# jasperlinthorst/reveal

Hardware: AMD Instinct MI355X
Metric: Mbp/s indexed+MUM-anchored (reveal rem) (higher is better)
Workload: dtype int32

## Files before the change

include/reveal_amd.h:

```cpp
#ifndef REVEAL_AMD_H
#define REVEAL_AMD_H
#include <stdint.h>

#ifdef __cplusplus
extern "C" {
#endif

typedef struct rv_index rv_index;

const char *rv_last_error(void);
int  rv_abi_version(void);
int  rv_sa_bits(void);
int  rv_device_count(void);

rv_index *rv_new(int device);
void rv_free(rv_index *h);

int rv_add_sample(rv_index *h);
int rv_add_sequence(rv_index *h, const char *seq, int64_t len, int64_t *begin, int64_t *end);
int rv_reset(rv_index *h);
int rv_reserve_text(rv_index *h, int64_t bytes);
int64_t rv_n(const rv_index *h);
int rv_nsamples(const rv_index *h);
int rv_nnodes(const rv_index *h);
int rv_add_sequences(rv_index *h, const char *text, int64_t total, const int64_t *lens, int64_t count);
int rv_node_list(const rv_index *h, int64_t *begin_end);

int rv_construct(rv_index *h, int rc, const char *safile, const char *lcpfile, int cache);
int rv_upload(rv_index *h);
int rv_upload_again(rv_index *h);

enum { RV_T = 0, RV_SA = 1, RV_SAI = 2, RV_LCP = 3, RV_SO = 4, RV_NSEP = 5, RV_NODES = 6 };
int64_t rv_get_array(rv_index *h, int which, void *out, int64_t cap);

int64_t rv_getmums(rv_index *h, int minl);
int rv_fetch_mums(rv_index *h, uint32_t *l, int64_t *a, int64_t *b, int64_t cap);
int64_t rv_getmultimums(rv_index *h, int minlength, int minn, int mems, int64_t *members);
int rv_fetch_multi(rv_index *h, uint32_t *l, int32_t *n, int64_t *off, uint16_t *so, int64_t *pos);

typedef struct {
    int64_t n;
    int32_t depth;
    int32_t nsamples;
    int32_t nnodes;
    int32_t parent;
    int32_t kind;
    int32_t reserved;
    int64_t nmums;
    int64_t nmembers;
} rv_sub;

int rv_align_begin(rv_index *h, int minl, int minn);
int rv_frontier_size(rv_index *h);
int rv_frontier_scan(rv_index *h);
int rv_sub_skip_scan(rv_index *h, int s);
int rv_sub_info(rv_index *h, int s, rv_sub *out);
int rv_sub_nodes(rv_index *h, int s, int64_t *begin_end );
int rv_sub_mums(rv_index *h, int s, uint32_t *l, int32_t *n, int64_t *off, uint16_t *so, int64_t *pos);
int64_t rv_sub_array(rv_index *h, int s, int which, void *out, int64_t cap);
int rv_sub_split(rv_index *h, int s, uint32_t l, int nsp, const int64_t *sp,
                 const int64_t *lead, int nlead, const int64_t *trail, int ntrail,
                 const int64_t *match, int nmatch, const int64_t *rest, int nrest);
int rv_frontier_commit(rv_index *h, int32_t *children);
int rv_align_end(rv_index *h);

typedef struct {
    int64_t steps;
    int64_t splits;
    int64_t anchored_bp;
    int32_t levels;
    int32_t maxdepth;
    int64_t scanned_ranks;
    double  t_scan, t_host, t_split, t_bubble;
} rv_align_stats;
int rv_align_builtin(rv_index *h, int minl, int minn, rv_align_stats *st);

int rv_align_builtin_until(rv_index *h, int minl, int minn, int stop_subs, rv_align_stats *st);
int rv_align_builtin_resume(rv_index *h, rv_align_stats *st);
int rv_align_builtin_continue(rv_index *h, int stop_subs, rv_align_stats *st);
int rv_frontier_counts(rv_index *h, int64_t *out);
int rv_frontier_export(rv_index *h, int64_t *meta, int64_t *node_first, int64_t *nodes);
int64_t rv_frontier_pack(rv_index *h, const int32_t *subs, int k, void *sa, void *lcp, void *bwt, int on_device);
int rv_frontier_import(rv_index *h, int minl, int minn, uint32_t maxlcp, int level, int nsubs, const int64_t *meta,
                       const int64_t *node_first, const int64_t *nodes, int64_t m,
                       const void *sa, const void *lcp, const void *bwt, int on_device);
int64_t rv_frontier_seeds_export(rv_index *h, const int32_t *subs, int k, int64_t *out, int64_t cap);
int rv_frontier_seeds_import(rv_index *h, int nsubs, const int64_t *words, int64_t nwords);
uint32_t rv_maxlcp(const rv_index *h);
int rv_cascade_info(const rv_index *h, int64_t *out);
const char *rv_cascade_why(const rv_index *h);
int64_t rv_anchor_count(rv_index *h, int64_t *members);
int rv_fetch_anchors(rv_index *h, uint32_t *l, int64_t *off, int64_t *pos);
int rv_set_result_buffers(rv_index *h, uint32_t *l, int64_t l_cap, int64_t *off, int64_t off_cap, int64_t *pos, int64_t pos_cap);
typedef struct {
    int64_t  key, n;
    int32_t  depth, nsamples, nnodes, picked;
    int64_t  nmums;
    uint32_t l; int32_t mn;
    int64_t  sp_min;
    uint64_t h_sa, h_lcp, h_mums;
} rv_trace;
int rv_set_trace(rv_index *h, int on);
int rv_set_preselect(rv_index *h, int64_t maxmums);
int rv_set_option(rv_index *h, const char *name, int64_t value);
int rv_get_option(rv_index *h, const char *name, int64_t *value);
int rv_set_launch_trace(int on);
int rv_option_count(void);
const char *rv_option_name(int k);
int64_t rv_trace_count(rv_index *h);
int rv_fetch_trace(rv_index *h, rv_trace *out, int64_t cap);

typedef struct rv_subindex rv_subindex;
rv_index *rv_clone(rv_index *h);
rv_subindex *rv_sx_main(rv_index *h);
rv_subindex *rv_sx_copy(rv_subindex *x);
void rv_sx_free(rv_subindex *x);
int rv_sx_info(const rv_subindex *x, rv_sub *out);
int rv_sx_nodes(const rv_subindex *x, int64_t *begin_end);
int64_t rv_sx_array(rv_subindex *x, int which, void *out, int64_t cap);
int64_t rv_sx_scan(rv_subindex *x, int minl, int minn, int64_t *members);
int rv_sx_fetch(rv_subindex *x, uint32_t *l, int32_t *n, int64_t *off, uint16_t *so, int64_t *pos);
int rv_sx_split(rv_subindex *x, const int64_t *lead, int nlead, const int64_t *trail, int ntrail,
                const int64_t *match, int nmatch, const int64_t *rest, int nrest, rv_subindex **out);
int rv_sx_extract(rv_subindex *x, int64_t *intervals, int niv);

int64_t rv_chain(int64_t m, int k, const uint32_t *len, const int32_t *nmem, const int64_t *crd, const int64_t *left,
                 const int64_t *right, int64_t wscore, int64_t wpen, int model, int64_t *out_idx, int64_t *out_score);

typedef struct { int64_t wscore, wpen, maxmums, seedsize; int gcmodel; int trim; double pcutoff; } rv_picker_args;
typedef struct {
    int picked; uint32_t pick_l; int32_t pick_n; int pick_members; uint16_t *pick_so; int64_t *pick_pos; int64_t member_cap;
    int64_t nleft, nright, nseed_members, seed_cap, seed_member_cap;
    uint32_t *seed_l; int32_t *seed_n; int64_t *seed_off; uint16_t *seed_so; int64_t *seed_pos; int64_t *seed_score; uint8_t *seed_right;
} rv_picker_out;
int rv_set_picker(rv_index *h, int kind, const rv_picker_args *args);
int rv_picker_info(const rv_index *h, int64_t *out);
int rv_pick_chain(const rv_picker_args *args, int nsub, int64_t m, const uint32_t *l, const int32_t *n, const int64_t *off, const uint16_t *so,
                  const int64_t *pos, int nsamples, const int64_t *seq_begin, const int64_t *iv_begin, const int64_t *iv_end, int minlength,
                  rv_picker_out *out);

typedef struct rv_graph rv_graph;
rv_graph *rv_graph_import(int64_t nnodes, const int64_t *node_b, const int64_t *node_e, const int8_t *node_aligned, const int8_t *node_sent,
                          const int64_t *off_ptr, const int32_t *off_sid, const int64_t *off_val,
                          int64_t nedges, const int32_t *edge_u, const int32_t *edge_v, const int64_t *edge_ptr, const int32_t *edge_paths,
                          const int64_t *pred_ptr, const int32_t *pred_edge, int npaths, const uint8_t *star, const int64_t *id2end,
                          int nstart, const int32_t *start_nodes, int literal_segments);
int rv_graph_pick(rv_graph *g, const rv_picker_args *args, int nsub, int64_t m, const uint32_t *l, const int32_t *n, const int64_t *off, const uint16_t *so, const int64_t *pos,
                  const int64_t *left, const int64_t *right, int minlength, rv_picker_out *out);
int rv_graph_align(rv_graph *g, const int64_t *nodes, int64_t nn, const int64_t *left, const int64_t *right, uint32_t l, const int64_t *pos, int npos,
                   int64_t *counts, int64_t *out6);
int rv_graph_align_fetch(rv_graph *g, int64_t *out);
int rv_set_graph_picker(rv_index *h, rv_graph *g, const rv_picker_args *args);
rv_graph *rv_graph_new(void);
int rv_graph_add_linear(rv_graph *g, int64_t b, int64_t e, int star);
int64_t rv_graph_read_gfa(rv_graph *g, rv_index *h, int64_t *text_n, const char *data, int64_t len, const char **names);
typedef struct GfaParsed rv_gfa_parsed;
rv_gfa_parsed *rv_gfa_parse(const char *data, int64_t len);
int64_t rv_graph_adopt(rv_graph *g, rv_index *h, int64_t *text_n, rv_gfa_parsed *parsed, const char **names);
void rv_gfa_parsed_free(rv_gfa_parsed *parsed);
int rv_graph_seal(rv_graph *g);
int rv_graph_paths(const rv_graph *g, int64_t *id2end);
int rv_graph_node_kinds(const rv_graph *g, int8_t *out);
int rv_graph_literal(const rv_graph *g);
int rv_graph_finish(rv_graph *g);
rv_graph *rv_graph_replay_begin(int nseq, const int64_t *begin, const int64_t *end);
int rv_set_replay_graph(rv_index *h, rv_graph *g);
rv_graph *rv_graph_replay(int nseq, const int64_t *begin, const int64_t *end, int64_t na, const uint32_t *an_l, const int64_t *an_off, const int64_t *an_pos);
const char *rv_graph_error(const rv_graph *g);
int rv_graph_sizes(const rv_graph *g, int64_t *out);
int rv_graph_export(const rv_graph *g, int64_t *node_b, int64_t *node_e, int8_t *node_aligned, int64_t *off_ptr, int32_t *off_sid, int64_t *off_val,
                    int64_t *succ_ptr, int32_t *succ_to, int32_t *succ_edge, int64_t *pred_ptr, int32_t *pred_from, int32_t *pred_edge, int64_t *edge_ptr, int32_t *edge_paths);
int rv_graph_prune(rv_graph *g, const char *T);
int64_t rv_graph_gfa(rv_graph *g, const char *T, int npaths, const char *const *names, const char *cmdline, const char **out);
void rv_graph_free(rv_graph *g);

enum { RV_K_SCAN_PAIR = 0, RV_K_SCAN_MULTI = 1, RV_K_SA_SORT = 2, RV_K_LCP = 3, RV_K_SPLIT = 4, RV_K_LABEL = 5,
       RV_K_BUBBLE = 6,
       RV_K_RADIX_SCATTER = 7, RV_K_RADIX_HIST = 8, RV_K_TEXT_ROUND = 9,
       RV_K_CASCADE = 10,
       RV_K_DIAG_TABLE = 11,
       RV_K_INIT_KEYS = 12,
       RV_K_PUBLISH = 13,
       RV_K_COUNT = 14 };
int rv_prof_enable(rv_index *h, int on);
int rv_prof_reset(rv_index *h);
int rv_prof_get(rv_index *h, int k, int64_t *launches, double *ms, double *bytes);
typedef struct rv_batch rv_batch;
rv_batch *rv_batch_new(void);
int rv_batch_add(rv_batch *b, rv_index *h);
int rv_batch_run(rv_batch *b, int minl, int minn, int construct, rv_align_stats *stats, int *status);
int rv_batch_info(const rv_batch *b, int64_t *out);
void rv_batch_free(rv_batch *b);
typedef struct rv_many rv_many;
rv_many *rv_many_new(int device);
void rv_many_free(rv_many *m);
int rv_many_option(rv_many *m, const char *name, int64_t value);
int64_t rv_many_add(rv_many *m, const char *const *seqs, const int64_t *lens, int k);
int rv_many_clear(rv_many *m);
int rv_many_run(rv_many *m, int minl, int minn, rv_align_stats *total);
int64_t rv_many_anchor_count(rv_many *m, int64_t *first, int64_t *members);
int rv_many_fetch(rv_many *m, uint32_t *l, int64_t *off, int64_t *pos);
int64_t rv_many_text(rv_many *m, int64_t job, char *out, int64_t cap);
int rv_many_info(const rv_many *m, int64_t *out);
int64_t rv_many_arrays(rv_many *m, int64_t job, int which, void *out, int64_t cap);
void *rv_dev_alloc(int device, int64_t bytes);
int rv_dev_free(int device, void *p);
int rv_ipc_export(int device, const void *p, uint8_t handle[64]);
void *rv_ipc_open(int device, const uint8_t handle[64]);
int rv_ipc_close(int device, void *p);
int rv_dev_copy(int device, void *dst, const void *src, int64_t bytes);
int rv_measure_bandwidth(int device, int64_t bytes, int iters, double *read_gbs, double *copy_gbs);
int rv_sa_stats(rv_index *h, int *sigma, int *bits, int *k0, int *rounds, int64_t *sorted_elems, int *radix_passes);
int rv_sa_diag_table(rv_index *h);
int rv_sa_tail(rv_index *h, int64_t *out);

int rv_test_exclusive_sum_u32(const uint32_t *in, uint32_t *out, int64_t n);
int rv_test_inclusive_max_u32(const uint32_t *in, uint32_t *out, int64_t n);
int rv_test_radix_sort(uint64_t *keys, uint32_t *vals, int64_t n, int bit_lo, int bit_hi);
int rv_test_radix_time(int64_t n, int bits, int dist, int flags, int iters, double *ms, int64_t *bad);

#ifdef __cplusplus
}
#endif
#endif
```

reveal_amd/_lib.py:

```python
import ctypes
import importlib.util
import os
import sys
import numpy as np

_HERE = os.path.dirname(os.path.abspath(__file__))

RV_T, RV_SA, RV_SAI, RV_LCP, RV_SO, RV_NSEP, RV_NODES = range(7)
K_SCAN_PAIR, K_SCAN_MULTI, K_SA_SORT, K_LCP, K_SPLIT, K_LABEL, K_BUBBLE, K_RADIX_SCATTER, K_RADIX_HIST, K_TEXT_ROUND, K_CASCADE, K_DIAG_TABLE, K_INIT_KEYS, K_PUBLISH = range(14)

c_i64p = ctypes.POINTER(ctypes.c_int64)
V = ctypes.c_void_p


class RvSub(ctypes.Structure):
    _fields_ = [("n", ctypes.c_int64), ("depth", ctypes.c_int32), ("nsamples", ctypes.c_int32),
                ("nnodes", ctypes.c_int32), ("parent", ctypes.c_int32), ("kind", ctypes.c_int32),
                ("reserved", ctypes.c_int32), ("nmums", ctypes.c_int64), ("nmembers", ctypes.c_int64)]


class RvAlignStats(ctypes.Structure):
    _fields_ = [("steps", ctypes.c_int64), ("splits", ctypes.c_int64), ("anchored_bp", ctypes.c_int64),
                ("levels", ctypes.c_int32), ("maxdepth", ctypes.c_int32), ("scanned_ranks", ctypes.c_int64),
                ("t_scan", ctypes.c_double), ("t_host", ctypes.c_double), ("t_split", ctypes.c_double),
                ("t_bubble", ctypes.c_double)]


TRACE_DTYPE = np.dtype([("key", np.int64), ("n", np.int64), ("depth", np.int32), ("nsamples", np.int32),
                        ("nnodes", np.int32), ("picked", np.int32), ("nmums", np.int64), ("l", np.uint32),
                        ("mn", np.int32), ("sp_min", np.int64), ("h_sa", np.uint64), ("h_lcp", np.uint64),
                        ("h_mums", np.uint64)], align=True)

_I, _L, _D = ctypes.c_int, ctypes.c_int64, ctypes.c_double
SYMBOLS = {
    "rv_last_error": (ctypes.c_char_p, []),
    "rv_abi_version": (_I, []),
    "rv_sa_bits": (_I, []),
    "rv_device_count": (_I, []),
    "rv_new": (V, [_I]),
    "rv_free": (None, [V]),
    "rv_add_sample": (_I, [V]),
    "rv_add_sequence": (_I, [V, ctypes.c_char_p, _L, c_i64p, c_i64p]),
    "rv_reset": (_I, [V]),
    "rv_reserve_text": (_I, [V, _L]),
    "rv_n": (_L, [V]),
    "rv_nsamples": (_I, [V]),
    "rv_nnodes": (_I, [V]),
    "rv_node_list": (_I, [V, V]),
    "rv_construct": (_I, [V, _I, ctypes.c_char_p, ctypes.c_char_p, _I]),
    "rv_upload": (_I, [V]),
    "rv_upload_again": (_I, [V]),
    "rv_get_array": (_L, [V, _I, V, _L]),
    "rv_getmums": (_L, [V, _I]),
    "rv_fetch_mums": (_I, [V, V, V, V, _L]),
    "rv_getmultimums": (_L, [V, _I, _I, _I, c_i64p]),
    "rv_fetch_multi": (_I, [V, V, V, V, V, V]),
    "rv_align_begin": (_I, [V, _I, _I]),
    "rv_frontier_size": (_I, [V]),
    "rv_frontier_scan": (_I, [V]),
    "rv_sub_skip_scan": (_I, [V, _I]),
    "rv_sub_info": (_I, [V, _I, ctypes.POINTER(RvSub)]),
    "rv_sub_nodes": (_I, [V, _I, V]),
    "rv_sub_mums": (_I, [V, _I, V, V, V, V, V]),
    "rv_sub_array": (_L, [V, _I, _I, V, _L]),
    "rv_sub_split": (_I, [V, _I, ctypes.c_uint32, _I, V, V, _I, V, _I, V, _I, V, _I]),
    "rv_frontier_commit": (_I, [V, V]),
    "rv_align_end": (_I, [V]),
    "rv_align_builtin": (_I, [V, _I, _I, ctypes.POINTER(RvAlignStats)]),
    "rv_align_builtin_until": (_I, [V, _I, _I, _I, ctypes.POINTER(RvAlignStats)]),
    "rv_align_builtin_resume": (_I, [V, ctypes.POINTER(RvAlignStats)]),
    "rv_align_builtin_continue": (_I, [V, _I, ctypes.POINTER(RvAlignStats)]),
    "rv_frontier_counts": (_I, [V, V]),
    "rv_frontier_export": (_I, [V, V, V, V]),
    "rv_frontier_pack": (_L, [V, V, _I, V, V, V, _I]),
    "rv_frontier_import": (_I, [V, _I, _I, ctypes.c_uint32, _I, _I, V, V, V, _L, V, V, V, _I]),
    "rv_frontier_seeds_export": (_L, [V, V, _I, V, _L]),
    "rv_frontier_seeds_import": (_I, [V, _I, V, _L]),
    "rv_maxlcp": (ctypes.c_uint32, [V]),
    "rv_cascade_info": (ctypes.c_int, [V, V]),
    "rv_cascade_why": (ctypes.c_char_p, [V]),
    "rv_anchor_count": (_L, [V, c_i64p]),
    "rv_fetch_anchors": (_I, [V, V, V, V]),
    "rv_set_result_buffers": (_I, [V, V, _L, V, _L, V, _L]),
    "rv_set_trace": (_I, [V, _I]),
    "rv_set_preselect": (_I, [V, _L]),
    "rv_set_option": (_I, [V, ctypes.c_char_p, _L]),
    "rv_set_launch_trace": (_I, [_I]),
    "rv_batch_new": (V, []),
    "rv_batch_add": (_I, [V, V]),
    "rv_batch_run": (_I, [V, _I, _I, _I, V, V]),
    "rv_batch_info": (_I, [V, V]),
    "rv_batch_free": (None, [V]),
    "rv_dev_alloc": (V, [_I, _L]),
    "rv_dev_free": (_I, [_I, V]),
    "rv_ipc_export": (_I, [_I, V, V]),
    "rv_ipc_open": (V, [_I, V]),
    "rv_ipc_close": (_I, [_I, V]),
    "rv_dev_copy": (_I, [_I, V, V, _L]),
    "rv_get_option": (_I, [V, ctypes.c_char_p, c_i64p]),
    "rv_option_count": (_I, []),
    "rv_option_name": (ctypes.c_char_p, [_I]),
    "rv_trace_count": (_L, [V]),
    "rv_fetch_trace": (_I, [V, V, _L]),
    "rv_clone": (V, [V]),
    "rv_sx_main": (V, [V]),
    "rv_sx_copy": (V, [V]),
    "rv_sx_free": (None, [V]),
    "rv_sx_info": (_I, [V, ctypes.POINTER(RvSub)]),
    "rv_sx_nodes": (_I, [V, V]),
    "rv_sx_array": (_L, [V, _I, V, _L]),
    "rv_sx_scan": (_L, [V, _I, _I, c_i64p]),
    "rv_sx_fetch": (_I, [V, V, V, V, V, V]),
    "rv_sx_split": (_I, [V, V, _I, V, _I, V, _I, V, _I, V]),
    "rv_sx_extract": (_I, [V, V, _I]),
    "rv_chain": (_L, [_L, _I, V, V, V, V, V, _L, _L, _I, V, V]),
    "rv_prof_enable": (_I, [V, _I]),
    "rv_prof_reset": (_I, [V]),
    "rv_prof_get": (_I, [V, _I, c_i64p, ctypes.POINTER(_D), ctypes.POINTER(_D)]),
    "rv_measure_bandwidth": (_I, [_I, _L, _I, ctypes.POINTER(_D), ctypes.POINTER(_D)]),
    "rv_sa_stats": (_I, [V] + [ctypes.POINTER(_I)] * 4 + [c_i64p, ctypes.POINTER(_I)]),
    "rv_sa_diag_table": (_I, [V]),
    "rv_sa_tail": (_I, [V, c_i64p]),
    "rv_set_picker": (_I, [V, _I, V]),
    "rv_picker_info": (_I, [V, c_i64p]),
    "rv_pick_chain": (_I, [V, _I, _L, V, V, V, V, V, _I, V, V, V, _I, V]),
    "rv_graph_import": (V, [_L, V, V, V, V, V, V, V, _L, V, V, V, V, V, V, _I, V, V, _I, V, _I]),
    "rv_graph_pick": (_I, [V, V, _I, _L, V, V, V, V, V, V, V, _I, V]),
    "rv_graph_align": (_I, [V, V, _L, V, V, ctypes.c_uint32, V, _I, V, V]),
    "rv_graph_align_fetch": (_I, [V, V]),
    "rv_graph_finish": (_I, [V]),
    "rv_set_graph_picker": (_I, [V, V, V]),
    "rv_graph_new": (V, []),
    "rv_graph_replay_begin": (V, [_I, V, V]),
    "rv_set_replay_graph": (_I, [V, V]),
    "rv_graph_add_linear": (_I, [V, _L, _L, _I]),
    "rv_graph_read_gfa": (_L, [V, V, V, V, _L, V]),
    "rv_graph_paths": (_I, [V, V]),
    "rv_graph_seal": (_I, [V]),
    "rv_gfa_parse": (V, [V, _L]),
    "rv_graph_adopt": (_L, [V, V, V, V, V]),
    "rv_gfa_parsed_free": (None, [V]),
    "rv_add_sequences": (_I, [V, V, _L, V, _L]),
    "rv_graph_node_kinds": (_I, [V, V]),
    "rv_graph_literal": (_I, [V]),
    "rv_graph_replay": (V, [_I, V, V, _L, V, V, V]),
    "rv_graph_error": (ctypes.c_char_p, [V]),
    "rv_graph_sizes": (_I, [V, c_i64p]),
    "rv_graph_export": (_I, [V] * 15),
    "rv_graph_prune": (_I, [V, V]),
    "rv_graph_gfa": (_L, [V, V, _I, V, V, V]),
    "rv_graph_free": (None, [V]),
    "rv_many_new": (V, [_I]),
    "rv_many_free": (None, [V]),
    "rv_many_option": (_I, [V, ctypes.c_char_p, _L]),
    "rv_many_add": (_L, [V, V, V, _I]),
    "rv_many_clear": (_I, [V]),
    "rv_many_run": (_I, [V, _I, _I, ctypes.POINTER(RvAlignStats)]),
    "rv_many_anchor_count": (_L, [V, V, c_i64p]),
    "rv_many_fetch": (_I, [V, V, V, V]),
    "rv_many_text": (_L, [V, _L, V, _L]),
    "rv_many_info": (_I, [V, V]),
    "rv_many_arrays": (_L, [V, _L, _I, V, _L]),
    "rv_test_exclusive_sum_u32": (_I, [V, V, _L]),
    "rv_test_inclusive_max_u32": (_I, [V, V, _L]),
    "rv_test_radix_sort": (_I, [V, V, _L, _I, _I]),
    "rv_test_radix_time": (_I, [_L, _I, _I, _I, _I, ctypes.POINTER(_D), c_i64p]),
}


def _share_torch_runtime():
    if os.environ.get("RV_SYSTEM_HIP") or "torch" in sys.modules:
        return
    try:
        spec = importlib.util.find_spec("torch")
    except (ImportError, ValueError):
        spec = None
    if spec is None or not spec.origin:
        return
    path = os.path.join(os.path.dirname(spec.origin), "lib", "libamdhip64.so")
    if os.path.exists(path):
        ctypes.CDLL(path, mode=ctypes.RTLD_GLOBAL)


class Lib:
    def __init__(self, sa64=False):
        self.sa64 = sa64
        _share_torch_runtime()
        name = "libreveal_amd64.so" if sa64 else "libreveal_amd.so"
        self.path = os.path.join(os.environ.get("RV_LIB_DIR") or _HERE, name)
        if not os.path.exists(self.path):
            raise ImportError("%s is missing: build it with `python -c 'import __graft_entry__ as g; g.build()'` "
                              "(hipcc --offload-arch=gfx950); reveal_amd has no CPU fallback" % self.path)
        self.dll = ctypes.CDLL(self.path)
        for sym, (res, args) in SYMBOLS.items():
            fn = getattr(self.dll, sym)
            fn.restype, fn.argtypes = res, args
        self.sa_t = np.int64 if sa64 else np.int32
        self.lcp_t = np.uint32 if sa64 else np.int32
        assert self.dll.rv_sa_bits() == (64 if sa64 else 32)
        v = os.environ.get("RV_LAUNCH_TRACE")
        if v is not None and v.strip() not in ("", "0"):
            self.dll.rv_set_launch_trace(1)

    def err(self):
        return (self.dll.rv_last_error() or b"").decode(errors="replace")


_libs = {}
_device = 0


def set_device(i):
    global _device
    _device = int(i)


def device():
    return _device


def measure_bandwidth(nbytes=1 << 30, iters=10):
    lib = get(False)
    r, c = _D(0), _D(0)
    if lib.dll.rv_measure_bandwidth(device(), int(nbytes), int(iters), ctypes.byref(r), ctypes.byref(c)) != 0:
        raise RuntimeError(lib.err())
    return r.value, c.value


def set_launch_trace(on=True):
    return [bool(get(w).dll.rv_set_launch_trace(1 if on else 0)) for w in (False, True)]


def get(sa64=False):
    if sa64 not in _libs:
        _libs[sa64] = Lib(sa64)
    return _libs[sa64]
```

reveal_amd/csrc/rv_api.hip:

```cpp
#include "rv_index.h"
#include "rv_cascade.h"
#include <limits>
#include <stdarg.h>
#include <stdio.h>
#include <string.h>
#include <limits.h>
#include <algorithm>
#include <thread>

static thread_local char g_err[1024] = "";

void rv_set_error(const char *fmt, ...) {
    va_list ap;
    va_start(ap, fmt);
    vsnprintf(g_err, sizeof g_err, fmt, ap);
    va_end(ap);
}

static std::vector<rv_index *> &live_handles() { static std::vector<rv_index *> v; return v; }
std::mutex &rv_trim_mutex() { static std::mutex *m = new std::mutex(); return *m; }
bool rv_oom_trim() {
    size_t got = 0;
    bool log = false;
    int caller_dev = 0;
// ... 844 lines not shown
int64_t rv_getmums(rv_index *h, int minl) {
    if (!h->constructed || h->main_arrays_freed) { rv_set_error("Index not yet constructed."); return -2; }
    (void)hipSetDevice(h->device);
    std::vector<RvPairRec> recs;
    if (rv_run_pair_scan(h, h->dSA.as<sa_t>(), h->dLCP.as<lcp_t>(), h->dBWT.as<uint8_t>(), h->n, minl, recs, nullptr, nullptr, nullptr, 0, nullptr, false) != 0) return -1;
    h->m_l.resize(recs.size()); h->m_a.resize(recs.size()); h->m_b.resize(recs.size());
    for (size_t k = 0; k < recs.size(); k++) {
        int64_t b = recs[k].b;
        if (h->rc == 1) b = h->nsep[0] + (h->nT - b - (int64_t)recs[k].l);
        h->m_l[k] = recs[k].l; h->m_a[k] = recs[k].a; h->m_b[k] = b;
    }
    return (int64_t)recs.size();
}

int rv_fetch_mums(rv_index *h, uint32_t *l, int64_t *a, int64_t *b, int64_t cap) {
    if (cap < (int64_t)h->m_l.size()) { rv_set_error("buffer too small"); return -1; }
    for (size_t k = 0; k < h->m_l.size(); k++) { l[k] = h->m_l[k]; a[k] = h->m_a[k]; b[k] = h->m_b[k]; }
    return 0;
}

int rv_prof_enable(rv_index *h, int on) {
    h->prof.on = on != 0;
    h->prof.mask = (on & 1) ? 0xFFFFFFFFu : ((u32)on >> 1);
    return 0;
}
int rv_prof_reset(rv_index *h) { (void)hipStreamSynchronize(h->ws.stream); h->prof.reset(); return 0; }
int rv_prof_get(rv_index *h, int k, int64_t *launches, double *ms, double *bytes) {
    if (k < 0 || k >= RV_K_COUNT) { rv_set_error("bad kernel id"); return -1; }
    (void)hipStreamSynchronize(h->ws.stream);
    h->prof.resolve();
    if (launches) *launches = h->prof.launches[k];
    if (ms) *ms = h->prof.ms[k];
    if (bytes) *bytes = h->prof.bytes[k];
    return 0;
}
int rv_sa_stats(rv_index *h, int *sigma, int *bits, int *k0, int *rounds, int64_t *sorted_elems, int *radix_passes) {
    if (sigma) *sigma = h->sa_stats.sigma;
    if (bits) *bits = h->sa_stats.bits;
    if (k0) *k0 = h->sa_stats.k0;
    if (rounds) *rounds = h->sa_stats.rounds;
    if (sorted_elems) *sorted_elems = h->sa_stats.sorted_elems;
    if (radix_passes) *radix_passes = h->sa_stats.radix_passes;
    return 0;
}
int rv_sa_diag_table(rv_index *h) { return h->sa_stats.diag_table; }
int rv_sa_tail(rv_index *h, int64_t *out) { if (!h || !out) return -1; out[0] = h->sa_stats.far_pairs; out[1] = h->sa_stats.lcp_list; return 0; }

}
namespace {
typedef int bw_v4 __attribute__((ext_vector_type(4)));
__global__ __launch_bounds__(256) void k_bw_read(const bw_v4 *__restrict__ a, int64_t n16, unsigned *sink) {
    bw_v4 acc = {0, 0, 0, 0};
    for (int64_t i = (int64_t)blockIdx.x * 256 + threadIdx.x; i < n16; i += (int64_t)gridDim.x * 256) acc ^= __builtin_nontemporal_load(a + i);
    if ((acc.x ^ acc.y ^ acc.z ^ acc.w) == 0x12345678) sink[0] = 1;
}
__global__ __launch_bounds__(256) void k_bw_copy(const bw_v4 *__restrict__ a, bw_v4 *__restrict__ b, int64_t n16) {
    for (int64_t i = (int64_t)blockIdx.x * 256 + threadIdx.x; i < n16; i += (int64_t)gridDim.x * 256) __builtin_nontemporal_store(__builtin_nontemporal_load(a + i), b + i);
}
}
extern "C" {
struct rv_batch {
    std::vector<rv_index *> hs;
    RvBatchGroup *g = nullptr;
    std::vector<std::string> errs;
};
rv_batch *rv_batch_new(void) {
    try { return new rv_batch(); } catch (...) { rv_set_error("rv_batch_new: out of host memory"); return nullptr; }
}
int rv_batch_add(rv_batch *b, rv_index *h) {
    if (!b || !h) { rv_set_error("rv_batch_add: null argument"); return -1; }
    if (!b->hs.empty() && b->hs[0]->device != h->device) { rv_set_error("rv_batch_add: the handles of a batch live on one device"); return -1; }
    try { b->hs.push_back(h); } catch (...) { rv_set_error("rv_batch_add: out of host memory"); return -1; }
    return 0;
}
void rv_batch_free(rv_batch *b) {
    if (!b) return;
    rv_batch_group_free(b->g);
    delete b;
}
int rv_batch_info(const rv_batch *b, int64_t *out) {
    out[0] = out[1] = 0;
    if (b && b->g) rv_batch_group_info(b->g, out);
    return 0;
}
int rv_batch_run(rv_batch *b, int minl, int minn, int construct, rv_align_stats *stats, int *status) {
    if (!b || b->hs.empty()) { rv_set_error("rv_batch_run: empty batch"); return -1; }
    const int n = (int)b->hs.size();
    try {
        b->errs.assign((size_t)n, std::string());
        if (!b->g) b->g = rv_batch_group_new(b->hs[0]->device);
        int members = 0;
        for (rv_index *h : b->hs) {
            const bool in = h->nsamples > 2 && !h->ws.opt.no_cascade;
            h->batch = in ? b->g : nullptr; h->batch_settled = false;
            members += in ? 1 : 0;
        }
        rv_batch_group_begin(b->g, members);
        std::vector<int> rc((size_t)n, 0);
        auto work = [&](int i) {
            rv_index *h = b->hs[(size_t)i];
            int r = 0;
            if (hipSetDevice(h->device) != hipSuccess) { rv_set_error("hipSetDevice failed"); r = -1; }
            if (r == 0 && construct) r = rv_construct(h, 0, "", "", 0);
            if (r == 0) r = rv_align_builtin(h, minl, minn, stats ? &stats[i] : nullptr);
            if (h->batch && !h->batch_settled) { h->batch_settled = true; rv_batch_group_leave(h->batch); }
            if (r != 0) b->errs[(size_t)i] = rv_last_error();
            rc[(size_t)i] = r;
        };
        std::vector<std::thread> th;
        int started = n;
        for (int i = 1; i < n; i++) {
            try { th.emplace_back(work, i); }
            catch (...) { started = i; break; }
        }
        if (started < n) for (int i = started; i < n; i++) { rv_index *h = b->hs[(size_t)i]; if (h->batch) { h->batch_settled = true; rv_batch_group_leave(h->batch); h->batch = nullptr; } }
        work(0);
        for (auto &t : th) t.join();
        for (int i = started; i < n; i++) work(i);
        int bad = -1;
        for (int i = 0; i < n; i++) { b->hs[(size_t)i]->batch = nullptr; if (status) status[i] = rc[(size_t)i]; if (rc[(size_t)i] != 0 && bad < 0) bad = i; }
        if (bad >= 0) { rv_set_error("rv_batch_run: job %d: %s", bad, b->errs[(size_t)bad].c_str()); return -1; }
        return 0;
    } catch (const std::exception &e) {
        for (rv_index *h : b->hs) h->batch = nullptr;
        rv_set_error("rv_batch_run: %s", e.what());
        return -1;
    }
}

void *rv_dev_alloc(int device, int64_t bytes) {
    void *p = nullptr;
    if (bytes < 0 || hipSetDevice(device) != hipSuccess) { rv_set_error("rv_dev_alloc: bad device or size"); return nullptr; }
    const hipError_t e = hipMalloc(&p, (size_t)std::max<int64_t>(bytes, 256));
    if (e != hipSuccess) { (void)hipGetLastError(); rv_set_error("rv_dev_alloc(%lld bytes): %s", (long long)bytes, hipGetErrorString(e)); return nullptr; }
    return p;
}
int rv_dev_free(int device, void *p) {
    if (!p) return 0;
    RV_HIP(hipSetDevice(device));
    RV_HIP(hipFree(p));
    return 0;
}
int rv_ipc_export(int device, const void *p, uint8_t handle[64]) {
    static_assert(sizeof(hipIpcMemHandle_t) == 64, "hipIpcMemHandle_t is 64 bytes");
    RV_HIP(hipSetDevice(device));
    hipIpcMemHandle_t hd;
    RV_HIP(hipIpcGetMemHandle(&hd, const_cast<void *>(p)));
    memcpy(handle, &hd, 64);
    return 0;
}
void *rv_ipc_open(int device, const uint8_t handle[64]) {
    if (hipSetDevice(device) != hipSuccess) { rv_set_error("rv_ipc_open: bad device"); return nullptr; }
    hipIpcMemHandle_t hd;
    memcpy(&hd, handle, 64);
    void *p = nullptr;
    const hipError_t e = hipIpcOpenMemHandle(&p, hd, hipIpcMemLazyEnablePeerAccess);
    if (e != hipSuccess) { (void)hipGetLastError(); rv_set_error("rv_ipc_open: %s", hipGetErrorString(e)); return nullptr; }
    return p;
}
int rv_ipc_close(int device, void *p) {
    if (!p) return 0;
    RV_HIP(hipSetDevice(device));
    RV_HIP(hipIpcCloseMemHandle(p));
    return 0;
}
int rv_dev_copy(int device, void *dst, const void *src, int64_t bytes) {
    if (bytes <= 0) return 0;
    RV_HIP(hipSetDevice(device));
    RV_HIP(hipMemcpy(dst, src, (size_t)bytes, hipMemcpyDefault));
    RV_HIP(hipStreamSynchronize(nullptr));
    return 0;
}

int rv_measure_bandwidth(int device, int64_t bytes, int iters, double *read_gbs, double *copy_gbs) {
    if (bytes < (1 << 20) || iters < 1) { rv_set_error("rv_measure_bandwidth: bytes >= 1 MiB and iters >= 1 needed"); return -1; }
    RV_HIP(hipSetDevice(device));
    const int64_t n16 = bytes / 16;
    void *a = nullptr, *b = nullptr; unsigned *sink = nullptr;
    hipStream_t q = nullptr; hipEvent_t e0 = nullptr, e1 = nullptr;
    RV_HIP(hipMalloc(&a, (size_t)n16 * 16)); RV_HIP(hipMalloc(&b, (size_t)n16 * 16)); RV_HIP(hipMalloc((void **)&sink, 64));
    RV_HIP(hipStreamCreateWithFlags(&q, hipStreamNonBlocking));
    RV_HIP(hipEventCreate(&e0)); RV_HIP(hipEventCreate(&e1));
    RV_HIP(hipMemsetAsync(a, 1, (size_t)n16 * 16, q)); RV_HIP(hipMemsetAsync(b, 2, (size_t)n16 * 16, q));
    const unsigned grid = 256 * 16;
    double out[2] = {0, 0};
    for (int pass = 0; pass < 2; pass++) {
        for (int r = -1; r < iters; r++) {
            if (r == 0) RV_HIP(hipEventRecord(e0, q));
            if (pass == 0) hipLaunchKernelGGL(k_bw_read, dim3(grid), dim3(256), 0, q, (const bw_v4 *)a, n16, sink);
            else hipLaunchKernelGGL(k_bw_copy, dim3(grid), dim3(256), 0, q, (const bw_v4 *)a, (bw_v4 *)b, n16);
        }
        RV_HIP(hipEventRecord(e1, q));
        RV_HIP(hipEventSynchronize(e1));
        float ms = 0.f;
        RV_HIP(hipEventElapsedTime(&ms, e0, e1));
        out[pass] = (double)n16 * 16 * (pass ? 2 : 1) * iters / ((double)ms * 1e6);
    }
    if (read_gbs) *read_gbs = out[0];
    if (copy_gbs) *copy_gbs = out[1];
    (void)hipEventDestroy(e0); (void)hipEventDestroy(e1); (void)hipStreamDestroy(q);
    (void)hipFree(a); (void)hipFree(b); (void)hipFree(sink);
    return 0;
}

static int test_ws(Workspace &ws) {
    if (rv_device_count() <= 0) { rv_set_error("no HIP device"); return -1; }
    RV_HIP(hipSetDevice(0));
    RV_HIP(hipStreamCreateWithFlags(&ws.stream, hipStreamNonBlocking));
    return 0;
}
static void test_ws_done(Workspace &ws) { ws.release(); (void)hipStreamDestroy(ws.stream); }

static int test_scan(const uint32_t *in, uint32_t *out, int64_t n, bool maxscan) {
    Workspace ws;
    RV_TRY(test_ws(ws));
    DBuf a, b;
    int r = 0;
    if (a.reserve((size_t)n * 4 + 64) || b.reserve((size_t)n * 4 + 64)) r = -1;
    if (!r && hipMemcpy(a.p, in, (size_t)n * 4, hipMemcpyHostToDevice) != hipSuccess) r = -1;
    if (!r) r = maxscan ? rv_inclusive_max_u32(ws, a.as<u32>(), b.as<u32>(), n) : rv_exclusive_sum_u32(ws, a.as<u32>(), b.as<u32>(), n);
    if (!r && hipStreamSynchronize(ws.stream) != hipSuccess) { rv_set_error("sync failed: %s", hipGetErrorString(hipGetLastError())); r = -1; }
    if (!r && hipMemcpy(out, b.p, (size_t)n * 4, hipMemcpyDeviceToHost) != hipSuccess) r = -1;
    a.release(); b.release();
    test_ws_done(ws);
    return r;
}
int rv_test_exclusive_sum_u32(const uint32_t *in, uint32_t *out, int64_t n) { return test_scan(in, out, n, false); }
int rv_test_inclusive_max_u32(const uint32_t *in, uint32_t *out, int64_t n) { return test_scan(in, out, n, true); }

int rv_test_radix_sort(uint64_t *keys, uint32_t *vals, int64_t n, int bit_lo, int bit_hi) {
    Workspace ws;
    RV_TRY(test_ws(ws));
    DBuf k0, k1, v0, v1;
    int r = 0, in1 = 0;
    if (k0.reserve((size_t)n * 8 + 64) || k1.reserve((size_t)n * 8 + 64) || v0.reserve((size_t)n * 4 + 64) || v1.reserve((size_t)n * 4 + 64)) r = -1;
    if (!r && hipMemcpy(k0.p, keys, (size_t)n * 8, hipMemcpyHostToDevice) != hipSuccess) r = -1;
    if (!r && hipMemcpy(v0.p, vals, (size_t)n * 4, hipMemcpyHostToDevice) != hipSuccess) r = -1;
    if (!r) r = rv_radix_sort_pairs<u32>(ws, k0.as<u64>(), v0.as<u32>(), k1.as<u64>(), v1.as<u32>(), n, bit_lo, bit_hi, &in1);
    if (!r && hipStreamSynchronize(ws.stream) != hipSuccess) { rv_set_error("sync failed: %s", hipGetErrorString(hipGetLastError())); r = -1; }
    if (!r && hipMemcpy(keys, in1 ? k1.p : k0.p, (size_t)n * 8, hipMemcpyDeviceToHost) != hipSuccess) r = -1;
    if (!r && hipMemcpy(vals, in1 ? v1.p : v0.p, (size_t)n * 4, hipMemcpyDeviceToHost) != hipSuccess) r = -1;
    k0.release(); k1.release(); v0.release(); v1.release();
    test_ws_done(ws);
    return r;
}

}
namespace {
__device__ inline u64 rt_mix(u64 x) { x ^= x >> 33; x *= 0xff51afd7ed558ccdull; x ^= x >> 33; x *= 0xc4ceb9fe1a85ec53ull; x ^= x >> 33; return x; }
__global__ __launch_bounds__(256) void k_rt_fill(u64 *keys, u32 *vals, int64_t n, int bits, int dist) {
    const int64_t i = (int64_t)blockIdx.x * 256 + threadIdx.x;
    if (i >= n) return;
    u64 r = rt_mix((u64)i * 0x9E3779B97F4A7C15ull + 12345);
    u64 k = 0;
    if (dist == 0) k = r;
    else if (dist == 1) { u64 r2 = rt_mix(r); for (int j = 0; j < 17; j++) { k = k * 5 + 1 + (r2 & 3); r2 >>= 2; } }
    const u64 mask = bits >= 64 ? ~0ull : (1ull << bits) - 1;
    keys[i] = (k & mask) | (r & ~mask & 0x00ffffffffffffffull);
    vals[i] = (u32)i;
}
__global__ __launch_bounds__(256) void k_rt_check(const u64 *keys, const u32 *vals, int64_t n, int bits, unsigned long long *bad) {
    const int64_t i = (int64_t)blockIdx.x * 256 + threadIdx.x;
    if (i + 1 >= n) return;
    const u64 mask = bits >= 64 ? ~0ull : (1ull << bits) - 1;
    const u64 a = keys[i] & mask, b = keys[i + 1] & mask;
    if (a > b || (a == b && vals[i] > vals[i + 1])) atomicAdd(bad, 1ull);
}
}
extern "C" {
int rv_test_radix_time(int64_t n, int bits, int dist, int flags, int iters, double *ms, int64_t *bad) {
    Workspace ws;
    RV_TRY(test_ws(ws));
    ws.opt.rs_bits = (flags & 1) ? 10 : 8; ws.opt.rs_xcd = (flags & 2) ? 1 : 0; ws.opt.rs_cnt16 = (flags & 4) ? 1 : 0; ws.opt.rs_no_digit_bytes = (flags & 8) ? 1 : 0;
    DBuf k0, k1, v0, v1, db;
    int r = 0, in1 = 0;
    hipEvent_t e0 = nullptr, e1 = nullptr;
    if (k0.reserve((size_t)n * 8 + 64) || k1.reserve((size_t)n * 8 + 64) || v0.reserve((size_t)n * 4 + 64) || v1.reserve((size_t)n * 4 + 64) || db.reserve(64)) r = -1;
    if (!r && (hipEventCreate(&e0) != hipSuccess || hipEventCreate(&e1) != hipSuccess)) r = -1;
    for (int it = 0; !r && it < iters; it++) {
        hipLaunchKernelGGL(k_rt_fill, dim3((unsigned)ceil_div(n, 256)), dim3(256), 0, ws.stream, k0.as<u64>(), v0.as<u32>(), n, bits, dist);
        (void)hipEventRecord(e0, ws.stream);
        r = rv_radix_sort_pairs<u32>(ws, k0.as<u64>(), v0.as<u32>(), k1.as<u64>(), v1.as<u32>(), n, 0, bits, &in1);
        (void)hipEventRecord(e1, ws.stream);
        if (!r && hipEventSynchronize(e1) != hipSuccess) { rv_set_error("sync failed: %s", hipGetErrorString(hipGetLastError())); r = -1; }
        float t = 0;
        if (!r) { (void)hipEventElapsedTime(&t, e0, e1); ms[it] = t; }
    }
    if (!r) {
        (void)hipMemsetAsync(db.p, 0, 8, ws.stream);
        hipLaunchKernelGGL(k_rt_check, dim3((unsigned)ceil_div(n, 256)), dim3(256), 0, ws.stream, (const u64 *)(in1 ? k1.p : k0.p), (const u32 *)(in1 ? v1.p : v0.p), n, bits,
                           db.as<unsigned long long>());
        unsigned long long b = 0;
        if (hipMemcpyAsync(&b, db.p, 8, hipMemcpyDeviceToHost, ws.stream) != hipSuccess || hipStreamSynchronize(ws.stream) != hipSuccess) r = -1;
        *bad = (int64_t)b;
    }
    if (e0) (void)hipEventDestroy(e0);
    if (e1) (void)hipEventDestroy(e1);
    k0.release(); k1.release(); v0.release(); v1.release(); db.release();
    test_ws_done(ws);
    return r;
}

}
```

reveal_amd/csrc/rv_common.h:

```cpp
#pragma once
#include <mutex>
#include <thread>
#include <vector>
#include <utility>
#include <hip/hip_runtime.h>
#include <stdint.h>
#include <string.h>
#include <stddef.h>
#include <vector>
#include <string>

#ifdef RV_SA64
typedef int64_t  sa_t;
typedef uint32_t lcp_t;
#else
typedef int32_t  sa_t;
typedef int32_t  lcp_t;
#endif

typedef unsigned long long u64;
typedef unsigned int       u32;

void rv_set_error(const char *fmt, ...);

#define RV_HIP(x)                                                                              \
    do {                                                                                       \
        hipError_t e_ = (x);                                                                   \
        if (e_ != hipSuccess) {                                                                \
            rv_set_error("%s:%d %s: %s", __FILE__, __LINE__, #x, hipGetErrorString(e_));       \
            return -1;                                                                         \
        }                                                                                      \
    } while (0)
#define RV_TRY(x)                                                                              \
    do {                                                                                       \
        int r_ = (x);                                                                          \
        if (r_ != 0) return r_;                                                                \
    } while (0)
#define RV_OPTION_LIST(X) \
    X(bubble_par_min, "RV_BUBBLE_PAR_MIN", -1) \
    X(presel_log, "RV_PRESEL_LOG", 0) \
    X(presel_host, "RV_PRESEL_HOST", 0) \
    X(leaf_acap, "RV_LEAF_ACAP", 256) \
    X(bubble_lds_always, "RV_BUBBLE_LDS_ALWAYS", 0) \
    X(no_early_bubble, "RV_NO_EARLY_BUBBLE", 0) \
    X(early_bubble_many, "RV_EARLY_BUBBLE_MANY", 0) \
    X(no_early_split, "RV_NO_EARLY_SPLIT", 0) \
    X(keep_dead, "RV_KEEP_DEAD", 0) \
    X(bubble_no_lds, "RV_BUBBLE_NO_LDS", 0) \
    X(bubble_no_join, "RV_BUBBLE_NO_JOIN", 0) \
    X(bubble_no_merge, "RV_BUBBLE_NO_MERGE", 0) \
    X(tables_memcpy, "RV_TABLES_MEMCPY", 0) \
    X(bubble_parent_scratch, "RV_BUBBLE_PARENT_SCRATCH", 0) \
    X(level_log, "RV_LEVEL_LOG", 0) \
    X(pb_two_pass, "RV_PB_TWO_PASS", 0) \
    X(no_leaf, "RV_NO_LEAF", 0) \
    X(leaf_prof, "RV_LEAF_PROF", 0) \
    X(no_cascade, "RV_NO_CASCADE", 0) \
    X(cascade_second, "RV_CASCADE_SECOND", 0) \
    X(cascade_danger, "RV_CASCADE_DANGER", 1) \
    X(cascade_second_off, "RV_CASCADE_SECOND_OFF", 0) \
    X(sync_block, "RV_SYNC_BLOCK", 0) \
    X(pb_refresh_tmin, "RV_PB_REFRESH_TMIN", 0) \
    X(cascade_log, "RV_CASCADE_LOG", 0) \
    X(cascade_danger_min, "RV_CASCADE_DANGER_MIN", 0) \
    X(cascade_batch, "RV_CASCADE_BATCH", 8) \
    X(lcp_by_rank, "RV_LCP_BY_RANK", 0) \
    X(no_tiny_sa, "RV_NO_TINY_SA", 0) \
    X(no_short_alphabet, "RV_NO_SHORT_ALPHABET", 0) \
    X(no_fused_lcp, "RV_NO_FUSED_LCP", 0) \
    X(no_diag, "RV_NO_DIAG", 0) \
    X(no_packed_text, "RV_NO_PACKED_TEXT", 0) \
    X(no_heads_fusion, "RV_NO_HEADS_FUSION", 0) \
    X(no_twin_collapse, "RV_NO_TWIN_COLLAPSE", 0) \
    X(no_far_twins, "RV_NO_FAR_TWINS", 0) \
    X(no_lcp_list, "RV_NO_LCP_LIST", 0) \
    X(no_text_jump, "RV_NO_TEXT_JUMP", 0) \
    X(far_table, "RV_FAR_TABLE", 0) \
    X(no_slow_class, "RV_NO_SLOW_CLASS", 0) \
    X(no_dwalk_blocks, "RV_NO_DWALK_BLOCKS", 0) \
    X(no_pub_twins, "RV_NO_PUB_TWINS", 0) \
    X(sa_no_text, "RV_SA_NO_TEXT", 0) \
    X(text_mode, "RV_TEXT_MODE", -1) \
    X(carry_ch, "RV_CARRY_CH", -1) \
    X(rs_bits, "RV_RS_BITS", 8) \
    X(rs_xcd, "RV_RS_XCD", 1) \
    X(rs_cnt16, "RV_RS_CNT16", 1) \
    X(rs_no_digit_bytes, "RV_RS_NO_DIGIT_BYTES", 0) \
    X(diag_table, "RV_DIAG_TABLE", -1) \
    X(no_cascade_chain, "RV_NO_CASCADE_CHAIN", 0) \
    X(casm_rank_count, "RV_CASM_RANK_COUNT", 0) \
    X(casm_big_min, "RV_CASM_BIG_MIN", -1) \
    X(casm_no_big, "RV_CASM_NO_BIG", 0) \
    X(casm_big_root, "RV_CASM_BIG_ROOT", 1 << 22) \
    X(casm_big_total, "RV_CASM_BIG_TOTAL", 1 << 26) \
    X(lock_any, "RV_LOCK_ANY", 0) \
    X(presel_dev_min, "RV_PRESEL_DEV_MIN", 65536) \
    X(scan_v1, "RV_SCAN_V1", 0) \
    X(pick_threads, "RV_PICK_THREADS", 0) \
    X(cascade_prio, "RV_CASCADE_PRIO", 0)
struct RvOptions {
#define RV_X_(f, name, def) int64_t f = def;
    RV_OPTION_LIST(RV_X_)
#undef RV_X_
    int64_t *find(const char *name) {
#define RV_X_(f, nm, def) if (strcmp(name, nm) == 0) return &f;
        RV_OPTION_LIST(RV_X_)
#undef RV_X_
        return nullptr;
    }
};
extern int g_rv_launch_trace;
static inline bool rv_launch_trace_on() { return g_rv_launch_trace != 0; }
#define RV_LAUNCH_CHECK()                                                                      \
    do {                                                                                       \
        RV_HIP(hipGetLastError());                                                             \
        if (rv_launch_trace_on()) {                                                            \
            fprintf(stderr, "launch %s:%d\n", __FILE__, __LINE__);                             \
            fflush(stderr);                                                                    \
            RV_HIP(hipDeviceSynchronize());                                                    \
        }                                                                                      \
    } while (0)

static inline int64_t ceil_div(int64_t a, int64_t b) { return (a + b - 1) / b; }

#define RV_BWT_SIDE 0x80u
#define RV_BWT_CHAR 0x7fu

#ifdef __HIPCC__
__device__ inline u32 rv_wave_min_u32(u32 v) {
    const int inf = -1;
    int x = (int)v, y;
#define RV_DPP_MIN(ctrl, rmask)                                                        \
    y = __builtin_amdgcn_update_dpp(inf, x, ctrl, rmask, 0xf, false);                  \
    x = (int)(((u32)y < (u32)x) ? (u32)y : (u32)x);
    RV_DPP_MIN(0xB1, 0xf)
    RV_DPP_MIN(0x4E, 0xf)
    RV_DPP_MIN(0x141, 0xf)
    RV_DPP_MIN(0x140, 0xf)
    RV_DPP_MIN(0x142, 0xa)
    RV_DPP_MIN(0x143, 0xc)
#undef RV_DPP_MIN
    return (u32)__builtin_amdgcn_readlane(x, 63);
}
#endif

#ifdef __HIPCC__
template <int CTRL, int ROWMASK> __device__ inline u32 rv_dpp_u32(u32 x) { return (u32)__builtin_amdgcn_update_dpp(0, (int)x, CTRL, ROWMASK, 0xf, false); }
#define RV_WAVE_SCAN_STEPS(STEP)                                                     \
    STEP(0x111, 0xf, (lane & 15) >= 1)                                               \
    STEP(0x112, 0xf, (lane & 15) >= 2)                                               \
    STEP(0x114, 0xf, (lane & 15) >= 4)                                               \
    STEP(0x118, 0xf, (lane & 15) >= 8)                                               \
    STEP(0x142, 0xa, (lane & 31) >= 16)                                              \
    STEP(0x143, 0xc, lane >= 32)
__device__ inline u64 rv_wave_max_u64(u64 v) {
#define RV_STEP_(CTRL, RM, TAKE) { const u64 t = ((u64)rv_dpp_u32<CTRL, RM>((u32)(v >> 32)) << 32) | rv_dpp_u32<CTRL, RM>((u32)v); v = t > v ? t : v; }
    RV_WAVE_SCAN_STEPS(RV_STEP_)
#undef RV_STEP_
    return ((u64)(u32)__builtin_amdgcn_readlane((int)(u32)(v >> 32), 63) << 32) | (u32)__builtin_amdgcn_readlane((int)(u32)v, 63);
}
__device__ inline u64 rv_wave_seg_max_u64(u32 seg, u64 v) {
    const int lane = threadIdx.x & 63;
    u32 lo = (u32)v, hi = (u32)(v >> 32);
#define RV_STEP_(CTRL, RM, TAKE) { const u32 os = rv_dpp_u32<CTRL, RM>(seg), ol = rv_dpp_u32<CTRL, RM>(lo), oh = rv_dpp_u32<CTRL, RM>(hi); \
                                   const bool up = (TAKE) && os == seg && (oh > hi || (oh == hi && ol > lo)); lo = up ? ol : lo; hi = up ? oh : hi; }
    RV_WAVE_SCAN_STEPS(RV_STEP_)
#undef RV_STEP_
    return ((u64)hi << 32) | lo;
}
__device__ inline u32 rv_wave_seg_max_u32(u32 seg, u32 v) {
    const int lane = threadIdx.x & 63;
#define RV_STEP_(CTRL, RM, TAKE) { const u32 os = rv_dpp_u32<CTRL, RM>(seg), ov = rv_dpp_u32<CTRL, RM>(v); v = ((TAKE) && os == seg && ov > v) ? ov : v; }
    RV_WAVE_SCAN_STEPS(RV_STEP_)
#undef RV_STEP_
    return v;
}
__device__ inline u32 rv_wave_incl_sum_u32(u32 v) {
    const int lane = threadIdx.x & 63;
#define RV_STEP_(CTRL, RM, TAKE) { const u32 t = rv_dpp_u32<CTRL, RM>(v); v += (TAKE) ? t : 0u; }
    RV_WAVE_SCAN_STEPS(RV_STEP_)
#undef RV_STEP_
    return v;
}
#endif

bool rv_oom_trim();

inline hipError_t rv_event_wait(hipEvent_t ev) {
    hipError_t e;
    for (int spins = 0; (e = hipEventQuery(ev)) == hipErrorNotReady; spins++) {
        if (spins < 64) { __builtin_ia32_pause(); continue; }
        if (spins < 640) { std::this_thread::yield(); continue; }
        return hipEventSynchronize(ev);
    }
    return e;
}

struct DBuf {
    void  *p = nullptr;
    size_t cap = 0;
    int reserve(size_t bytes) {
        if (bytes <= cap) return 0;
        if (p) { (void)hipFree(p); p = nullptr; cap = 0; }
        size_t want = bytes + (bytes >= ((size_t)256 << 20) ? bytes / 64 : bytes / 8) + 256;
        hipError_t e = hipMalloc(&p, want);
        if (e == hipErrorOutOfMemory) {
            (void)hipGetLastError();
            if (rv_oom_trim()) e = hipMalloc(&p, want);
            if (e == hipErrorOutOfMemory) { (void)hipGetLastError(); want = bytes + 256; e = hipMalloc(&p, want); }
        }
        if (e != hipSuccess) { p = nullptr; rv_set_error("%s:%d hipMalloc(%zu bytes): %s", __FILE__, __LINE__, want, hipGetErrorString(e)); return -1; }
        cap = want;
        return 0;
    }
    void release() { if (p) (void)hipFree(p); p = nullptr; cap = 0; }
    template <class T> T *as() const { return (T *)p; }
};

struct RvPools {
    std::mutex mu;
    std::vector<std::pair<int, hipStream_t>> streams;
    struct Pin { int dev; void *p; size_t cap; };
    std::vector<Pin> pinned;
    size_t pinned_bytes = 0;
};
inline RvPools &rv_pools() { static RvPools *p = new RvPools(); return *p; }
inline hipError_t rv_stream_get(hipStream_t *s) {
    int dev = 0; (void)hipGetDevice(&dev);
    {
        RvPools &P = rv_pools();
        std::lock_guard<std::mutex> g(P.mu);
        for (size_t k = P.streams.size(); k-- > 0;)
            if (P.streams[k].first == dev) { *s = P.streams[k].second; P.streams.erase(P.streams.begin() + (ptrdiff_t)k); return hipSuccess; }
    }
    return hipStreamCreateWithFlags(s, hipStreamNonBlocking);
}
inline void rv_stream_put(hipStream_t s) {
    if (!s) return;
    (void)hipStreamSynchronize(s);
    int dev = 0; (void)hipGetDevice(&dev);
    RvPools &P = rv_pools();
    {
        std::lock_guard<std::mutex> g(P.mu);
        if (P.streams.size() < 64) { P.streams.push_back({dev, s}); return; }
    }
    (void)hipStreamDestroy(s);
}
inline hipError_t rv_pinned_get(size_t bytes, void **p, size_t *cap) {
    int dev = 0; (void)hipGetDevice(&dev);
    {
        RvPools &P = rv_pools();
        std::lock_guard<std::mutex> g(P.mu);
        size_t best = (size_t)-1;
        for (size_t k = 0; k < P.pinned.size(); k++)
            if (P.pinned[k].dev == dev && P.pinned[k].cap >= bytes && P.pinned[k].cap <= 4 * bytes + (1u << 20) && (best == (size_t)-1 || P.pinned[k].cap < P.pinned[best].cap)) best = k;
        if (best != (size_t)-1) { *p = P.pinned[best].p; *cap = P.pinned[best].cap; P.pinned_bytes -= *cap; P.pinned.erase(P.pinned.begin() + (ptrdiff_t)best); return hipSuccess; }
    }
    const hipError_t e = hipHostMalloc(p, bytes, hipHostMallocDefault);
    if (e == hipSuccess) *cap = bytes;
    return e;
}
inline void rv_pinned_put(void *p, size_t cap) {
    if (!p) return;
    int dev = 0; (void)hipGetDevice(&dev);
    RvPools &P = rv_pools();
    {
        std::lock_guard<std::mutex> g(P.mu);
        if (cap <= ((size_t)64 << 20) && P.pinned_bytes + cap <= ((size_t)512 << 20) && P.pinned.size() < 256) { P.pinned.push_back({dev, p, cap}); P.pinned_bytes += cap; return; }
    }
    (void)hipHostFree(p);
}

struct HBuf {
    void  *p = nullptr;
    size_t cap = 0;
    int reserve(size_t bytes) {
        if (bytes <= cap) return 0;
        if (p) { (void)hipDeviceSynchronize(); rv_pinned_put(p, cap); p = nullptr; cap = 0; }
        size_t want = bytes + bytes / 2 + 4096;
        RV_HIP(rv_pinned_get(want, &p, &cap));
        return 0;
    }
    void release() { if (p) rv_pinned_put(p, cap); p = nullptr; cap = 0; }
    template <class T> T *as() const { return (T *)p; }
};

struct Workspace {
    hipStream_t stream = nullptr;
    RvOptions opt;
    DBuf scan_tmp[4];
    DBuf rs_hist;
    DBuf rs_digits;
    DBuf misc[20];
    DBuf sa[32];
    HBuf hpin;
    hipEvent_t ev_rb = nullptr;
    void *prof_ctx = nullptr;
    int (*prof_begin_fn)(void *, hipStream_t, int, double) = nullptr;
    void (*prof_end_fn)(void *, hipStream_t, int) = nullptr;
    int prof_begin(int k, double bytes) { return prof_begin_fn ? prof_begin_fn(prof_ctx, stream, k, bytes) : -1; }
    void prof_end(int id) { if (prof_end_fn && id >= 0) prof_end_fn(prof_ctx, stream, id); }
    bool sa_in_use = false;
    size_t trim_sa() {
        size_t got = 0;
        for (auto &b : sa) { got += b.cap; b.release(); }
        return got;
    }
    void release() {
        hpin.release();
        if (ev_rb) { (void)hipEventDestroy(ev_rb); ev_rb = nullptr; }
        for (auto &b : scan_tmp) b.release();
        rs_hist.release(); rs_digits.release();
        for (auto &b : misc) b.release();
        for (auto &b : sa) b.release();
    }
};

std::mutex &rv_trim_mutex();
struct SaScratchInUse {
    Workspace &w; bool was;
    SaScratchInUse(Workspace &x) : w(x) { std::lock_guard<std::mutex> g(rv_trim_mutex()); was = w.sa_in_use; w.sa_in_use = true; }
    ~SaScratchInUse() { std::lock_guard<std::mutex> g(rv_trim_mutex()); w.sa_in_use = was; }
};

int rv_exclusive_sum_u32(Workspace &ws, const u32 *in, u32 *out, int64_t n);
int rv_exclusive_sum_u64(Workspace &ws, const u64 *in, u64 *out, int64_t n);
int rv_inclusive_max_u32(Workspace &ws, const u32 *in, u32 *out, int64_t n);
int rv_inclusive_max_u64(Workspace &ws, const u64 *in, u64 *out, int64_t n);

int rv_radix_passes(const Workspace &ws, int nbits);
template <class V>
int rv_radix_sort_pairs(Workspace &ws, u64 *k0, V *v0, u64 *k1, V *v1, int64_t n,
                        int bit_lo, int bit_hi, int *result_in_1);

int rv_read_back(Workspace &ws, void *dst, const void *dsrc, size_t bytes);

int rv_h2d_copy(Workspace &ws, const void *pinned_src, void *dst, size_t bytes);

struct RvSaStats {
    int    sigma, bits, k0;
    int    rounds;
    int64_t sorted_elems;
    int    radix_passes;
    int    diag_table;
    int64_t far_pairs;
    int64_t lcp_list;
};
int rv_build_sa(Workspace &ws, const uint8_t *T, int64_t n, sa_t *SA, RvSaStats *st,
                lcp_t *LCP = nullptr, uint8_t *BWT = nullptr, sa_t side_sep = 0, u32 *d_maxlcp = nullptr, bool *fused_done = nullptr,
                const int64_t *seps = nullptr, int nseps = 0);
int rv_build_inverse(Workspace &ws, const sa_t *SA, sa_t *SAi, int64_t n);
int rv_build_inverse_checked(Workspace &ws, const sa_t *SA, sa_t *SAi, int64_t n);
int rv_build_lcp(Workspace &ws, const uint8_t *T, const sa_t *SA, bool by_rank, lcp_t *LCP, int64_t n, u32 *d_maxlcp, uint8_t *BWT, sa_t side_sep);
int rv_build_bwt(Workspace &ws, const uint8_t *T, const sa_t *SA, int64_t n, uint8_t *BWT, sa_t side_sep);
```

reveal_amd/csrc/rv_construct.hip:

```cpp
#include "rv_common.h"
#include <string.h>
#include <stdlib.h>
#include <algorithm>
#include <limits>

#ifdef RV_SA64
typedef u64 sav_t;
#else
typedef u32 sav_t;
#endif

namespace {

constexpr int TB = 256;

__device__ inline u64 swar_eq(u64 v, uint8_t c) {
    const u64 t = v ^ (0x0101010101010101ull * c);
    return ~(((t & 0x7f7f7f7f7f7f7f7full) + 0x7f7f7f7f7f7f7f7full) | t) & 0x8080808080808080ull;
}
__device__ inline u64 swar_acgt(u64 v) { return swar_eq(v, 'A') | swar_eq(v, 'C') | swar_eq(v, 'G') | swar_eq(v, 'T'); }
__device__ inline u32 swar_code2(u64 v) {
    u64 y = ((v >> 1) ^ (v >> 2)) & 0x0303030303030303ull;
    y = (y | (y >> 6)) & 0x000f000f000f000full;
    y = (y | (y >> 12)) & 0x000000ff000000ffull;
// ... 2013 lines not shown
                    if (x >= 8 && lim > 8) {
                        x = 8;
                        while (x + 8 <= lim) {
                            u64 a, b;
                            __builtin_memcpy(&a, txt + i + x, 8);
                            __builtin_memcpy(&b, txt + j + x, 8);
                            if (a != b) { x += __builtin_ctzll(a ^ b) >> 3; break; }
                            x += 8;
                        }
                        while (x < lim && txt[i + x] == txt[j + x]) x++;
                    }
                    j_less = (x < lim) ? (txt[j + x] < txt[i + x]) : (j > i);
                }
                cnt += j_less ? 1 : 0;
            }
            wj = (wj >> 8) | (nxt << 56);
            nxt >>= 8;
        }
    }
    ord[cnt] = (uint16_t)i;
}
__global__ __launch_bounds__(TB) void k_sa_tiny_emit(const uint8_t *__restrict__ T, int n, const uint16_t *__restrict__ ord, sa_t *__restrict__ SA, lcp_t *__restrict__ LCP,
                                                     uint8_t *__restrict__ BWT, sa_t side_sep, u32 *__restrict__ d_maxlcp) {
    __shared__ uint8_t txt[TINY_N + 16];
    for (int k = threadIdx.x; k < n + 16; k += TB) txt[k] = k < n ? T[k] : (uint8_t)0;
    __syncthreads();
    const int r = (int)blockIdx.x * TB + threadIdx.x;
    u32 l = 0;
    if (r < n) {
        const int i = ord[r];
        if (r > 0) {
            const int j = ord[r - 1];
            const int lim = n - (i > j ? i : j);
            int x = 0;
            while (x < lim) { const uint8_t c = txt[i + x]; if (c != txt[j + x] || c == '$' || c == 'N') break; x++; }
            l = (u32)x;
        }
        SA[r] = (sa_t)i; LCP[r] = (lcp_t)l;
        BWT[r] = (uint8_t)((i > 0 ? txt[i - 1] : (uint8_t)'$') | ((sa_t)i > side_sep ? RV_BWT_SIDE : 0u));
    }
    const u32 wm = (u32)rv_wave_max_u64((u64)l);
    if ((threadIdx.x & 63) == 0 && wm) atomicMax(d_maxlcp, wm);
}

inline int bitlen(u64 v) { int b = 0; while (v) { b++; v >>= 1; } return b; }

}

int rv_build_inverse(Workspace &ws, const sa_t *SA, sa_t *SAi, int64_t n) {
    if (n <= 0) return 0;
    hipLaunchKernelGGL(k_inverse, dim3((unsigned)ceil_div(n, TB)), dim3(TB), 0, ws.stream, SA, SAi, n);
    RV_LAUNCH_CHECK();
    return 0;
}

int rv_build_inverse_checked(Workspace &ws, const sa_t *SA, sa_t *SAi, int64_t n) {
    if (n <= 0) return 0;
    RV_TRY(ws.misc[1].reserve(64));
    u32 *d_err = ws.misc[1].as<u32>();
    RV_HIP(hipMemsetAsync(d_err, 0, 4, ws.stream));
    RV_HIP(hipMemsetAsync(SAi, 0xFF, (size_t)n * sizeof(sa_t), ws.stream));
    hipLaunchKernelGGL(k_inverse_checked, dim3((unsigned)ceil_div(n, TB)), dim3(TB), 0, ws.stream, SA, SAi, n, d_err);
    RV_LAUNCH_CHECK();
    hipLaunchKernelGGL(k_inverse_verify, dim3((unsigned)ceil_div(n, TB)), dim3(TB), 0, ws.stream, SA, (const sa_t *)SAi, n, d_err);
    RV_LAUNCH_CHECK();
    u32 err = 0;
    RV_TRY(rv_read_back(ws, &err, d_err, 4));
    if (err) { rv_set_error("the suffix array file does not hold a permutation of 0..n-1 (%s): stale or foreign cache file?", (err & 1u) ? "entry out of range" : "duplicate entries"); return -1; }
    return 0;
}

int rv_build_bwt(Workspace &ws, const uint8_t *T, const sa_t *SA, int64_t n, uint8_t *BWT, sa_t side_sep) {
    if (n <= 0) return 0;
    hipLaunchKernelGGL(k_bwt, dim3((unsigned)ceil_div(n, TB)), dim3(TB), 0, ws.stream, T, SA, n, BWT, side_sep);
    RV_LAUNCH_CHECK();
    return 0;
}

int rv_build_lcp(Workspace &ws, const uint8_t *T, const sa_t *SA, bool by_rank, lcp_t *LCP, int64_t n, u32 *d_maxlcp, uint8_t *BWT, sa_t side_sep) {
    SaScratchInUse in_use(ws);
    if (n <= 0) return 0;
    RV_HIP(hipMemsetAsync(d_maxlcp, 0, sizeof(u32), ws.stream));
    if (by_rank || ws.opt.lcp_by_rank) {
        hipLaunchKernelGGL(k_lcp, dim3((unsigned)ceil_div(n, TB)), dim3(TB), 0, ws.stream, T, SA, LCP, n, d_maxlcp, BWT, side_sep);
        RV_LAUNCH_CHECK();
        return 0;
    }
    DBuf &bphi = ws.sa[1], &bpl = ws.sa[0];
    RV_TRY(bphi.reserve((size_t)n * sizeof(sa_t)));
    RV_TRY(bpl.reserve((size_t)n * 8));
    hipLaunchKernelGGL(k_phi, dim3((unsigned)ceil_div(n, TB)), dim3(TB), 0, ws.stream, SA, n, bphi.as<sa_t>());
    RV_LAUNCH_CHECK();
    hipLaunchKernelGGL(k_plcp, dim3((unsigned)ceil_div(ceil_div(n, PHI_K), TB)), dim3(TB), 0, ws.stream, T, (const sa_t *)bphi.as<sa_t>(), bpl.as<u64>(), n, side_sep);
    RV_LAUNCH_CHECK();
    hipLaunchKernelGGL(k_lcp_gather, dim3((unsigned)ceil_div(n, TB)), dim3(TB), 0, ws.stream, SA, (const u64 *)bpl.as<u64>(), LCP, n, d_maxlcp, BWT);
    RV_LAUNCH_CHECK();
    return 0;
}

int rv_build_sa(Workspace &ws, const uint8_t *T, int64_t n, sa_t *SA, RvSaStats *st,
                lcp_t *LCP, uint8_t *BWT, sa_t side_sep, u32 *d_maxlcp, bool *fused_done, const int64_t *seps, int nseps) {
    SaScratchInUse in_use(ws);
    RvSaStats s;
    memset(&s, 0, sizeof s);
    if (fused_done) *fused_done = false;
    if (n <= 0) { if (st) *st = s; return 0; }
    if (n >= ((int64_t)1 << 32) - 2) { rv_set_error("SA build: n >= 2^32-2 not supported yet"); return -1; }
    hipStream_t q = ws.stream;
    if (n <= TINY_N / 2 && LCP && BWT && d_maxlcp && !ws.opt.no_tiny_sa) {
        RV_TRY(ws.sa[0].reserve((size_t)TINY_N * 2 + 64));
        RV_HIP(hipMemsetAsync(d_maxlcp, 0, sizeof(u32), q));
        const unsigned nb = (unsigned)ceil_div(n, TB);
        hipLaunchKernelGGL(k_sa_tiny_rank, dim3(nb), dim3(TB), 0, q, T, (int)n, ws.sa[0].as<uint16_t>());
        RV_LAUNCH_CHECK();
        hipLaunchKernelGGL(k_sa_tiny_emit, dim3(nb), dim3(TB), 0, q, T, (int)n, (const uint16_t *)ws.sa[0].as<uint16_t>(), SA, LCP, BWT, side_sep, d_maxlcp);
        RV_LAUNCH_CHECK();
        s.rounds = 0; s.sorted_elems = 0;
        if (st) *st = s;
        if (fused_done) *fused_done = true;
        return 0;
    }

    DBuf &d_hist = ws.sa[16], &d_lut = ws.sa[17];
    RV_TRY(d_hist.reserve(264 * sizeof(u32)));
    RV_TRY(d_lut.reserve(256));
    RV_HIP(hipMemsetAsync(d_hist.p, 0, 264 * sizeof(u32), q));
    {
        int64_t blocks = ceil_div(n, (int64_t)TB * 16);
        if (blocks > 2048) blocks = 2048;
        hipLaunchKernelGGL(k_hist256, dim3((unsigned)blocks), dim3(TB), 0, q, T, n, d_hist.as<u32>());
        RV_LAUNCH_CHECK();
    }
    u32 hist[257];
    RV_TRY(rv_read_back(ws, hist, d_hist.p, sizeof hist));
    uint8_t lut[256];
    int sigma = 0;
    for (int c = 0; c < 256; c++) lut[c] = hist[c] ? (uint8_t)(++sigma) : (uint8_t)0;
    u32 radix = (u32)sigma + 1;
    if (sigma >= 255) radix = 256;
    if (sigma >= 255) for (int c = 0; c < 256; c++) lut[c] = (uint8_t)c;
    const bool short_alphabet = sigma >= 2 && sigma < 255 && T != nullptr && hist[(uint8_t)'$'] > 0 && lut[(uint8_t)'$'] == 1 && hist[256] == 0 && !ws.opt.no_short_alphabet;
    bool ends_with_sep = false;
    if (short_alphabet) { uint8_t last = 0; RV_TRY(rv_read_back(ws, &last, T + (n - 1), 1)); ends_with_sep = last == (uint8_t)'$'; }
    if (short_alphabet && ends_with_sep) {
        for (int c = 0; c < 256; c++) lut[c] = hist[c] ? (uint8_t)(lut[c] - 1) : (uint8_t)0;
        radix = (u32)sigma;
    }
    int K = 1;
    int bits = 0;
    KeyPack kp;
    {
        const double base = sigma > 2 ? (double)(sigma - 1) : 2.0;
        const double want = (double)n * ((seps && nseps > 1) ? 16.0 : 1.0);
        int best_g = 0, best_K = 0, best_bits = 0;
        u64 rg = 1;
        for (int g = 1; g <= KP_MAXG; g++) {
            rg *= radix;
            if (rg > KP_MAXFIELD && g > 1) break;
            const int fb = bitlen(rg - 1);
            auto bits_of = [&](int k) { u64 rl = 1; for (int e = 0; e < k % g; e++) rl *= radix; return (k / g) * fb + (k % g ? bitlen(rl - 1) : 0); };
            bool exact = true;
            for (int i = 1; i < g && exact; i++) {
                u64 d = 1; for (int e = 0; e < g - i; e++) d *= radix;
                const u32 m = (u32)(((1ull << 20) + d - 1) / d);
                for (u64 f = 0; f < rg && exact; f++) exact = ((f * m) >> 20) == f / d && f * m < (1ull << 32);
            }
            if (!exact) continue;
            int k = 1; double cap = base;
            while (cap < want && bits_of(k + 1) <= 62) { cap *= base; k++; }
            const int passes = rv_radix_passes(ws, bits_of(k));
            while (bits_of(k + 1) <= 62 && rv_radix_passes(ws, bits_of(k + 1)) == passes) k++;
            const int b = bits_of(k);
            if (k > best_K || (k == best_K && b < best_bits)) { best_g = g; best_K = k; best_bits = b; }
        }
        K = best_K; bits = best_bits;
        u64 rgb = 1; for (int e = 0; e < best_g; e++) rgb *= radix;
        kp.g = best_g; kp.fb = bitlen(rgb - 1); kp.nf = (K + best_g - 1) / best_g; kp.gl = K - (kp.nf - 1) * best_g;
        u64 rl = 1; for (int e = 0; e < kp.gl; e++) rl *= radix;
        kp.fbl = bitlen(rl - 1); kp.bits = bits; kp.rad = radix; kp.fmask = (1u << kp.fb) - 1u; kp.lmask = (1u << kp.fbl) - 1u;
        kp.lscale = (u32)(rgb / rl); kp.fdiv = (1u << 16) / (u32)kp.fb + 1u;
        kp.lastmul = kp.gl == best_g ? (1u << 20) : (u32)(((1ull << 20) + kp.lscale - 1) / kp.lscale);
        for (int i = 1; i < KP_MAXG; i++) {
            u64 d = 1; for (int e = 0; e < best_g - i; e++) d *= radix;
            kp.dmul[i - 1] = i < best_g ? (u32)(((1ull << 20) + d - 1) / d) : 0u;
        }
    }
    s.sigma = sigma; s.bits = bits; s.k0 = K;
    RV_HIP(hipMemcpyAsync(d_lut.p, lut, 256, hipMemcpyHostToDevice, q));
    bool fused = LCP && BWT && d_maxlcp && bits <= 48 && !ws.opt.no_fused_lcp;
    KeyDigits kd;
    kd.ly.sortmask = bits >= 64 ? ~0ull : (1ull << bits) - 1;
    kd.ly.at_bits = K <= 30 ? 5 : 8; kd.ly.at_shift = 56 - kd.ly.at_bits;
    kd.ly.nd_shift = (bits + 7) / 8 * 8; kd.ly.nd_bits = 0;
    kd.D = (side_sep > 0 && (int64_t)side_sep < n - 1) ? (int64_t)side_sep + 1 : 0;
    kd.ns = 0;
    for (int q2 = 0; q2 < HINT_K - 1; q2++) kd.sep[q2] = std::numeric_limits<int64_t>::max();
    for (int q2 = 0; q2 < HINT_K; q2++) kd.Ds[q2] = 0;
    if (seps && nseps > 0 && kd.D > 0) {
        kd.ns = (nseps + 1 < HINT_K + 1) ? nseps + 1 : HINT_K + 1;
        if (kd.ns > HINT_K) kd.ns = HINT_K;
        for (int q2 = 0; q2 < kd.ns - 1; q2++) kd.sep[q2] = seps[q2];
        for (int q2 = 1; q2 < kd.ns; q2++) kd.Ds[q2] = seps[q2 - 1] + 1;
        if (nseps + 1 > HINT_K) kd.ns = 0;
    }
    const bool want_hint = fused && kd.D > 0 && kd.ns >= 2 && kd.ly.at_shift - kd.ly.nd_shift >= 8 && !ws.opt.no_diag && !ws.opt.no_packed_text;
    if (want_hint) kd.ly.nd_bits = std::min(kd.ly.at_shift - kd.ly.nd_shift - 1, 11);
    kd.K = K; kd.kp = kp; kd.stop0 = lut[(uint8_t)'$']; kd.stop1 = lut[(uint8_t)'N'];
    if (fused) RV_HIP(hipMemsetAsync(d_maxlcp, 0, sizeof(u32), q));

    DBuf &bk0 = ws.sa[0], &bk1 = ws.sa[1], &bv0 = ws.sa[2], &bv1 = ws.sa[3], &bhead = ws.sa[4], &bseed = ws.sa[5], &bgrp = ws.sa[6], &bisa = ws.sa[7],
         &bP0 = ws.sa[8], &bP1 = ws.sa[9], &bG0 = ws.sa[10], &bG1 = ws.sa[11], &btile = ws.sa[12], &bbig = ws.sa[13], &bQb = ws.sa[14], &bPb = ws.sa[15];
    auto freeall = [&]() {};
#define SA_TRY(x) do { int r__ = (x); if (r__) { freeall(); return r__; } } while (0)
#define SA_HIP(x) do { hipError_t e__ = (x); if (e__ != hipSuccess) { rv_set_error("%s:%d %s", __FILE__, __LINE__, hipGetErrorString(e__)); freeall(); return -1; } } while (0)
    SA_TRY(bk0.reserve((size_t)n * 8)); SA_TRY(bk1.reserve((size_t)n * 8));
    SA_TRY(bv0.reserve((size_t)n * sizeof(sav_t))); SA_TRY(bv1.reserve((size_t)n * sizeof(sav_t)));
    SA_TRY(bhead.reserve((size_t)n + 16));
    auto need_seed_grp = [&](int64_t cnt) -> int {
        RV_TRY(bseed.reserve((size_t)std::max<int64_t>(cnt, 1) * (sizeof(sav_t) > 4 ? sizeof(sav_t) : 4)));
        return bgrp.reserve((size_t)std::max<int64_t>(cnt, 1) * 4);
    };
    SA_TRY(bisa.reserve((size_t)n * 4));
    const unsigned nblk = (unsigned)ceil_div(n, TB);

    DiagBits dg; dg.stop = dg.exc = dg.lt = nullptr; dg.D = kd.D; dg.tab = 0;
    kd.dtab = nullptr;
    const int64_t nw = (n + 63) / 64;
    DiagSamples dsm; dsm.ns = kd.ns;
    for (int q2 = 0; q2 < HINT_K - 1; q2++) dsm.sep[q2] = kd.sep[q2];
    for (int q2 = 0; q2 < HINT_K; q2++) dsm.Ds[q2] = kd.Ds[q2];
    if (kd.ly.nd_bits > 0) {
        DBuf &bds = ws.sa[20], &bde = ws.sa[21], &bdl = ws.sa[22];
        SA_TRY(bds.reserve((size_t)nw * 8)); SA_TRY(bde.reserve((size_t)nw * 8)); SA_TRY(bdl.reserve((size_t)nw * 8));
        hipLaunchKernelGGL(k_diag_bits, dim3((unsigned)ceil_div(nw, TB)), dim3(TB), 0, q, T, n, dsm, bds.as<u64>(), bde.as<u64>(), bdl.as<u64>(), nw);
        SA_HIP(hipGetLastError());
        dg.stop = bds.as<u64>(); dg.exc = bde.as<u64>(); dg.lt = bdl.as<u64>();
    }
    const bool collapse = fused && kd.ly.nd_bits > 0 && kd.ns == 2 && K < 64 && kd.D > 1 && n > kd.D + 1 && !ws.opt.no_heads_fusion && !ws.opt.no_twin_collapse
                          && (sizeof(sav_t) > 4 || n < ((int64_t)1 << 31));
    int64_t nsort = n;
    const u32 *tw_off = nullptr;
    if (collapse) {
        const int64_t ntiles = ceil_div(n, KEY_TILE);
        DBuf &btw = ws.sa[23];
        SA_TRY(btw.reserve((size_t)(std::max<int64_t>(ntiles, ceil_div(n, TB)) + 1) * 4 + 64));
        u32 *tc = btw.as<u32>();
        auto count_kept = [&](int tab, u32 *kept_out) -> int {
            hipLaunchKernelGGL(k_tw_count, dim3((unsigned)ceil_div(nw, TB)), dim3(TB), 0, q, (const u64 *)dg.stop, nw, K, kd.D, n, tc, ntiles, tab);
            RV_LAUNCH_CHECK();
            RV_HIP(hipMemsetAsync(tc + ntiles, 0, 4, q));
            RV_TRY(rv_exclusive_sum_u32(ws, tc, tc, ntiles + 1));
            return rv_read_back(ws, kept_out, tc + ntiles, 4);
        };
        u32 kept = 0;
        SA_TRY(count_kept(0, &kept));
        const int dt_mode = (int)ws.opt.diag_table;
        const int64_t n2 = n - kd.D;
        if (dt_mode != 0 && n >= 4096 && (dt_mode == 1 || (int64_t)kept * 10 > n2 * 3)) {
            const int64_t mseeds = nw * SEED_SLOTS;
            DBuf &bdt = ws.sa[25];
            const int64_t ndt = (n >> DT_SHIFT) + 1;
            SA_TRY(bdt.reserve((size_t)ndt * 8 + 64));
            int32_t *raw = bdt.as<int32_t>(), *tab = raw + ndt;
            const int did = ws.prof_begin(11 , (double)n + (double)mseeds * 12.0);
            hipLaunchKernelGGL(k_seed_sample, dim3((unsigned)ceil_div(nw, TB)), dim3(TB), 0, q, T, n, bk0.as<u64>(), bv0.as<sav_t>(), nw);
            SA_HIP(hipGetLastError());
            int sin1 = 0;
            SA_TRY(rv_radix_sort_pairs<sav_t>(ws, bk0.as<u64>(), bv0.as<sav_t>(), bk1.as<u64>(), bv1.as<sav_t>(), mseeds, 0, 40, &sin1));
            SA_HIP(hipMemsetAsync(raw, 0x7f, (size_t)ndt * 4, q));
            hipLaunchKernelGGL(k_seed_pairs, dim3((unsigned)ceil_div(mseeds, TB)), dim3(TB), 0, q, (const u64 *)(sin1 ? bk1.as<u64>() : bk0.as<u64>()),
                               (const sav_t *)(sin1 ? bv1.as<sav_t>() : bv0.as<sav_t>()), mseeds, kd.D, kd.D, raw);
            SA_HIP(hipGetLastError());
            hipLaunchKernelGGL(k_dtab_fill, dim3((unsigned)ceil_div(ndt, TB)), dim3(TB), 0, q, T, n, kd.D, kd.D, (const int32_t *)raw, tab, ndt);
            SA_HIP(hipGetLastError());
            DiagTab dt; dt.dtab = tab; dt.S2 = kd.D; dt.D = kd.D;
            hipLaunchKernelGGL(k_diag_bits_tab, dim3((unsigned)ceil_div(nw, TB)), dim3(TB), 0, q, T, n, dt, ws.sa[20].as<u64>(), ws.sa[21].as<u64>(), ws.sa[22].as<u64>(), nw);
            SA_HIP(hipGetLastError());
            ws.prof_end(did);
            u32 kept_tab = 0;
            SA_TRY(count_kept(1, &kept_tab));
            if (dt_mode == 1 || (int64_t)kept_tab * 5 < (int64_t)kept * 4) { kept = kept_tab; kd.dtab = tab; dg.tab = 1; }
            else {
                hipLaunchKernelGGL(k_diag_bits, dim3((unsigned)ceil_div(nw, TB)), dim3(TB), 0, q, T, n, dsm, ws.sa[20].as<u64>(), ws.sa[21].as<u64>(), ws.sa[22].as<u64>(), nw);
                SA_HIP(hipGetLastError());
                SA_TRY(count_kept(0, &kept));
            }
        }
        nsort = kd.D + (int64_t)kept;
        tw_off = tc;
        s.diag_table = dg.tab;
    }
    {
        const int64_t iktiles = ceil_div(n, KEY_TILE);
        const dim3 ig((unsigned)std::min<int64_t>(iktiles, 256 * 8));
#define RV_IK_(G) hipLaunchKernelGGL(k_init_keys<G>, ig, dim3(TB), 0, q, T, n, d_lut.as<uint8_t>(), K, kp, bk0.as<u64>(), bv0.as<sav_t>(), fused ? 1 : 0, \
                                     kd.stop0, kd.stop1, kd.ly, dg, tw_off, iktiles)
        const int ikid = ws.prof_begin(12 , (double)n + (double)nsort * (8.0 + sizeof(sav_t) + 1.0));
        switch (kp.g) { case 1: RV_IK_(1); break; case 2: RV_IK_(2); break; case 3: RV_IK_(3); break; case 4: RV_IK_(4); break; default: RV_IK_(5); break; }
        ws.prof_end(ikid);
#undef RV_IK_
    }
    SA_HIP(hipGetLastError());
    int in1 = 0;
    SA_TRY(rv_radix_sort_pairs<sav_t>(ws, bk0.as<u64>(), bv0.as<sav_t>(), bk1.as<u64>(), bv1.as<sav_t>(), nsort, 0, bits, &in1));
    s.radix_passes += rv_radix_passes(ws, bits); s.sorted_elems += nsort;
    u64 *ks = in1 ? bk1.as<u64>() : bk0.as<u64>();
    sav_t *vs = in1 ? bv1.as<sav_t>() : bv0.as<sav_t>();
    u64 *kt = in1 ? bk0.as<u64>() : bk1.as<u64>();
    sav_t *vt = in1 ? bv0.as<sav_t>() : bv1.as<sav_t>();

    uint8_t *head = bhead.as<uint8_t>();
    if (!collapse) SA_TRY(need_seed_grp(n));
    u32 *seed = bseed.as<u32>(), *grp = bgrp.as<u32>(), *ISA = bisa.as<u32>();
    const u64 *keys_by_rank = ks;
    const sav_t *vals_by_rank = vs;
    if (collapse) {
        const int64_t nb = ceil_div(nsort, TC_TILE);
        u32 *bc = ws.sa[23].as<u32>();
        hipLaunchKernelGGL(k_tw_flags, dim3((unsigned)nb), dim3(TB), 0, q, (const sav_t *)vs, nsort, bc);
        SA_HIP(hipGetLastError());
        SA_TRY(rv_exclusive_sum_u32(ws, bc, bc, nb));
        sav_t *vexp = reinterpret_cast<sav_t *>(bisa.p);
        if (sizeof(sav_t) > 4) { SA_TRY(ws.sa[24].reserve((size_t)n * sizeof(sav_t))); vexp = ws.sa[24].as<sav_t>(); }
        const int pbid = ws.prof_begin(13 , (double)nsort * 2.0 * (8.0 + sizeof(sav_t)) + (double)n * (1.0 + sizeof(sa_t) + sizeof(lcp_t) + 1.0));
        hipLaunchKernelGGL(k_heads_publish_tc, dim3((unsigned)nb), dim3(TB), 0, q, (const u64 *)ks, (const sav_t *)vs, nsort, (const u32 *)bc, head, LCP, SA, BWT,
                           side_sep, kd, d_maxlcp, ws.opt.no_pub_twins ? 0 : 1, kt, vexp);
        ws.prof_end(pbid);
        SA_HIP(hipGetLastError());
        keys_by_rank = kt; vals_by_rank = vexp;
    } else if (fused && kd.ly.nd_bits > 0 && !ws.opt.no_heads_fusion) {
        hipLaunchKernelGGL(k_heads_publish, dim3((unsigned)ceil_div(n, (int64_t)HP_ITEMS * TB)), dim3(TB), 0, q, (const u64 *)ks, (const sav_t *)vs, n, head, seed, LCP, SA, BWT, side_sep, kd, d_maxlcp,
                           ws.opt.no_pub_twins ? 0 : 1);
        SA_HIP(hipGetLastError());
        SA_TRY(rv_inclusive_max_u32(ws, seed, grp, n));
    } else {
        hipLaunchKernelGGL(k_heads, dim3(nblk), dim3(TB), 0, q, (const u64 *)ks, n, head, seed, fused ? LCP : (lcp_t *)nullptr, kd, fused ? d_maxlcp : (u32 *)nullptr);
        SA_HIP(hipGetLastError());
        SA_TRY(rv_inclusive_max_u32(ws, seed, grp, n));
        {
            KeyDigits kp = kd;
            if (ws.opt.no_pub_twins) kp.ly.nd_bits = 0;
            hipLaunchKernelGGL(k_publish0, dim3(nblk), dim3(TB), 0, q, (const sav_t *)vs, n, SA, (const u64 *)ks, fused ? BWT : (uint8_t *)nullptr, side_sep,
                               kp, fused ? LCP : (lcp_t *)nullptr, head, d_maxlcp, grp);
        }
        SA_HIP(hipGetLastError());
    }
    bool isa_built = false;
    const sav_t *cur_S = nullptr; const u32 *cur_G = nullptr; int64_t cur_m = 0;
    auto need_isa = [&]() -> int {
        if (isa_built) return 0;
        hipLaunchKernelGGL(k_isa_identity, dim3(nblk), dim3(TB), 0, q, (const sa_t *)SA, n, ISA);
        RV_LAUNCH_CHECK();
        if (cur_m > 0) {
            hipLaunchKernelGGL(k_round_isa, dim3((unsigned)ceil_div(cur_m, TB)), dim3(TB), 0, q, cur_S, cur_G, cur_m, ISA);
            RV_LAUNCH_CHECK();
        }
        isa_built = true;
        return 0;
    };

    int64_t ntile = ceil_div(n, CP_TILE);
    SA_TRY(btile.reserve(std::max((size_t)(ntile + 1) * 8 + 64, (size_t)RT_REGIONS * 4)));
    u32 *tile = btile.as<u32>();
    auto count_unsorted = [&](const uint8_t *hd, int64_t len, int64_t *m_out) -> int {
        const int64_t nt = ceil_div(len, CP_TILE);
        hipLaunchKernelGGL(k_cp_count, dim3((unsigned)nt), dim3(TB), 0, q, hd, len, tile);
        RV_LAUNCH_CHECK();
        RV_HIP(hipMemsetAsync(tile + nt, 0, 4, q));
        RV_TRY(rv_exclusive_sum_u32(ws, tile, tile, nt + 1));
        u32 tot = 0;
        RV_TRY(rv_read_back(ws, &tot, tile + nt, 4));
        *m_out = tot;
        return 0;
    };
    auto emit_unsorted = [&](const uint8_t *hd, int64_t len, const u32 *pos_in, const sav_t *suf_in, const u32 *grp_in, u32 *P, sav_t *S, u32 *G,
                             const uint8_t *cls_in = nullptr, uint8_t *cls_out = nullptr, int cls_is = 0) -> int {
        const int64_t nt = ceil_div(len, CP_TILE);
        hipLaunchKernelGGL(k_cp_emit, dim3((unsigned)nt), dim3(TB), 0, q, hd, len, (const u32 *)tile, pos_in, suf_in, grp_in, P, S, G, cls_in, cls_out, cls_is);
        RV_LAUNCH_CHECK();
        return 0;
    };
    int64_t m = 0;
    if (collapse) {
        u32 *tlast = tile + (ntile + 1);
        hipLaunchKernelGGL(k_cp_count_g, dim3((unsigned)ntile), dim3(TB), 0, q, (const uint8_t *)head, n, tile, tlast);
        SA_HIP(hipGetLastError());
        SA_HIP(hipMemsetAsync(tile + ntile, 0, 4, q));
        SA_TRY(rv_exclusive_sum_u32(ws, tile, tile, ntile + 1));
        SA_TRY(rv_inclusive_max_u32(ws, tlast, tlast, ntile));
        u32 tot = 0;
        SA_TRY(rv_read_back(ws, &tot, tile + ntile, 4));
        m = tot;
        SA_TRY(bP0.reserve((size_t)std::max<int64_t>(m, 1) * 4)); SA_TRY(bG0.reserve((size_t)std::max<int64_t>(m, 1) * 4));
        SA_TRY(need_seed_grp(m));
        seed = bseed.as<u32>(); grp = bgrp.as<u32>();
        if (m > 0) {
            hipLaunchKernelGGL(k_cp_emit_g, dim3((unsigned)ntile), dim3(TB), 0, q, (const uint8_t *)head, n, (const u32 *)tile, (const u32 *)tlast, vals_by_rank,
                               bP0.as<u32>(), vt, bG0.as<u32>());
            SA_HIP(hipGetLastError());
        }
    } else {
        SA_TRY(count_unsorted(head, n, &m));
        SA_TRY(bP0.reserve((size_t)std::max<int64_t>(m, 1) * 4)); SA_TRY(bG0.reserve((size_t)std::max<int64_t>(m, 1) * 4));
        if (m > 0) SA_TRY(emit_unsorted(head, n, nullptr, vals_by_rank, grp, bP0.as<u32>(), vt, bG0.as<u32>()));
    }
    const int64_t m_list0 = m;
    u32 *P = bP0.as<u32>(), *G = bG0.as<u32>(), *Pn = nullptr, *Gn = nullptr;
    sav_t *S = vt;
    sav_t *Sfree = vs;
    u64 *kA = ks, *kB = kt;
    if (m > 0) { SA_TRY(bbig.reserve((size_t)m + 16)); SA_TRY(bQb.reserve((size_t)m * 4)); SA_TRY(bPb.reserve((size_t)m * 4)); }

    const int lowbits = bitlen((u64)n), highbits = bitlen((u64)(n > 1 ? n - 1 : 1));
    int64_t h = K;
    const bool can_far = fused && kd.ly.nd_bits > 0 && kd.ns == 2 && dg.stop != nullptr && !ws.opt.no_far_twins;
    const bool can_list = fused && !ws.opt.no_lcp_list;
    bool text_round_ran = false, far_ran = false, partial = false;
    DBuf &btodo = ws.sa[26];
    int64_t ntodo = 0;
    auto todo_add = [&](const u32 *ranks, int64_t cnt) -> int {
        if (cnt <= 0) return 0;
        if ((size_t)(ntodo + cnt) * 4 > btodo.cap) {
            DBuf nb;
            RV_TRY(nb.reserve((size_t)(ntodo + cnt) * 4 * 2 + 1024));
            if (ntodo) RV_HIP(hipMemcpyAsync(nb.p, btodo.p, (size_t)ntodo * 4, hipMemcpyDeviceToDevice, q));
            RV_HIP(hipStreamSynchronize(q));
            btodo.release();
            btodo = nb;
        }
        RV_HIP(hipMemcpyAsync(btodo.as<u32>() + ntodo, ranks, (size_t)cnt * 4, hipMemcpyDeviceToDevice, q));
        ntodo += cnt;
        return 0;
    };
    auto leave_fused = [&](const u32 *ranks, int64_t cnt) -> int {
        if (!fused) return 0;
        if (!can_list) { fused = false; return 0; }
        partial = true;
        return todo_add(ranks, cnt);
    };
    bool list_in_todo = false;
    DBuf &bcls0 = ws.sa[30], &bcls1 = ws.sa[31];
    uint8_t *cls = nullptr, *cls_next = nullptr;
    while (m > 0) {
        if (h >= 2 * n + 2 + 2 * TEXT_LIM) { rv_set_error("SA build: did not converge"); freeall(); return -1; }
        s.rounds++;
        const unsigned mb = (unsigned)ceil_div(m, TB);
        uint8_t *bigflag = bbig.as<uint8_t>();
        cur_S = S; cur_G = G; cur_m = m;
        const bool far_round = text_round_ran && !far_ran && can_far;
        const bool text_round = !far_round && s.rounds == 1 && h <= 64 && !ws.opt.sa_no_text;
        bool text_big = false;
        if (far_round) {
            far_ran = true;
            DBuf &bR = ws.sa[27], &bM = ws.sa[28];
            const int64_t nw1 = ceil_div(kd.D - 1, (int64_t)64);
            SA_TRY(bR.reserve(std::max((size_t)nw * 4 + 64, (size_t)(nw1 * 64 + 64) * 4))); SA_TRY(bM.reserve((size_t)nw * 4 + 64));
            hipLaunchKernelGGL(k_far_rev, dim3((unsigned)ceil_div(nw, TB)), dim3(TB), 0, q, (const u64 *)dg.stop, nw, bR.as<u32>());
            SA_HIP(hipGetLastError());
            SA_TRY(rv_inclusive_max_u32(ws, bR.as<u32>(), bM.as<u32>(), nw));
            FarTwins ft; ft.stop = dg.stop; ft.exc = dg.exc; ft.lt = dg.lt; ft.M = bM.as<u32>(); ft.nw = nw; ft.n = n; ft.S2 = kd.D; ft.D = kd.D; ft.dtab = kd.dtab;
            const bool nd_table = m >= ((int64_t)1 << 21) || ws.opt.far_table == 1;
            if (nd_table) {
                hipLaunchKernelGGL(k_far_nd, dim3((unsigned)ceil_div(nw1, TB)), dim3(TB), 0, q, ft, bR.as<u32>(), nw1);
                SA_HIP(hipGetLastError());
            }
            hipLaunchKernelGGL(k_far_twins, dim3(mb), dim3(TB), 0, q, T, S, (const u32 *)G, (const u32 *)P, m, ft, nd_table ? (const u32 *)bR.as<u32>() : (const u32 *)nullptr, head, bigflag, SA, LCP, BWT, side_sep, d_maxlcp);
            SA_HIP(hipGetLastError());
        }
        else if (text_round)
        {
            text_round_ran = true;
            FusedOut fo;
            fo.pk.Tp = nullptr; fo.pk.blk = nullptr;
            if (!ws.opt.no_packed_text) {
                DBuf &bTp = ws.sa[18], &bBlk = ws.sa[19];
                const int64_t nwords = n / 32 + 4, nblk = n / PK_BLOCK + 8;
                SA_TRY(bTp.reserve((size_t)(nwords + 8) * 8)); SA_TRY(bBlk.reserve((size_t)nblk + 16));
                SA_HIP(hipMemsetAsync(bBlk.p, 0, (size_t)nblk + 16, q));
                SA_HIP(hipMemsetAsync(bTp.as<u64>() + nwords, 0, 64, q));
                hipLaunchKernelGGL(k_pack2, dim3((unsigned)ceil_div(nwords, TB)), dim3(TB), 0, q, T, n, bTp.as<u64>(), bBlk.as<uint8_t>(), nwords);
                SA_HIP(hipGetLastError());
                fo.pk.Tp = bTp.as<u64>(); fo.pk.blk = bBlk.as<uint8_t>();
            }
            fo.LCP = fused ? LCP : (lcp_t *)nullptr; fo.BWT = BWT; fo.keys = keys_by_rank; fo.maxlcp = d_maxlcp; fo.side_sep = side_sep; fo.kd = kd;
            fo.h = (int)h;
            fo.far_defer = (can_far && kd.dtab == nullptr) ? 1 : 0;
            const int tmode = ws.opt.text_mode >= 0 ? (int)ws.opt.text_mode : (kd.ly.nd_bits > 0 ? 3 : 1);
#define RT_LAUNCH(M_) hipLaunchKernelGGL((k_round_text<4, M_>), dim3(mb), dim3(TB), 0, q, T, S, (const u32 *)G, (const u32 *)P, m, head, bigflag, SA, Sfree, fo)
            const int tid = ws.prof_begin(9 , (double)m * (4 + 4 + sizeof(sav_t) + 8) + (double)m * (sizeof(sav_t) + sizeof(sa_t) + sizeof(lcp_t) + 2));
            if (tmode == 3 && fused) {
                u32 *work = bQb.as<u32>(), *work_count = tile;
                const u32 reg_cap = (u32)(ceil_div((int64_t)mb, RT_REGIONS) * (TB / 2));
                SA_HIP(hipMemsetAsync(work_count, 0, RT_REGIONS * 4, q));
                hipLaunchKernelGGL((k_round_text3<4>), dim3(mb), dim3(TB), 0, q, T, S, (const u32 *)G, (const u32 *)P, m, n, head, bigflag, SA, Sfree, fo, work, work_count, reg_cap);
                SA_HIP(hipGetLastError());
                u32 cnt[RT_REGIONS];
                SA_TRY(rv_read_back(ws, cnt, work_count, sizeof cnt));
                u32 mx = 0;
                for (int r = 0; r < RT_REGIONS; r++) mx = std::max(mx, cnt[r]);
                if (mx) {
                    const u32 bpr = (u32)ceil_div((int64_t)mx, TB);
                    hipLaunchKernelGGL((k_round_text3b<4>), dim3(bpr * RT_REGIONS), dim3(TB), 0, q, T, S, (const u32 *)G, m, n, head, SA, fo, (const u32 *)work,
                                       (const u32 *)work_count, reg_cap, bpr);
                }
            }
            else if (tmode == 0) RT_LAUNCH(0); else if (tmode == 2) RT_LAUNCH(2); else RT_LAUNCH(1);
#undef RT_LAUNCH
            SA_HIP(hipGetLastError());
            ws.prof_end(tid);
            hipLaunchKernelGGL(k_medium_back, dim3((unsigned)ceil_div(m, (int64_t)TB * 8)), dim3(TB), 0, q, (const uint8_t *)bigflag, (const sav_t *)Sfree, S, m);
        }
        else {
            if (!list_in_todo) { SA_TRY(leave_fused(P, m)); list_in_todo = true; }
            SA_TRY(need_isa());
            const uint8_t *slow = (cls && 2 * h <= TEXT_LIM) ? cls : nullptr;
            hipLaunchKernelGGL(k_round_small, dim3(mb), dim3(TB), 0, q, S, (const u32 *)G, (const u32 *)P, m, n, h, (const u32 *)ISA, head, bigflag, SA, slow);
        }
        SA_HIP(hipGetLastError());
        if (!far_round) {
            const int64_t nt = ceil_div(m, CP_TILE);
            hipLaunchKernelGGL(k_flag_count, dim3((unsigned)nt), dim3(TB), 0, q, (const uint8_t *)bigflag, m, tile);
            SA_HIP(hipGetLastError());
            SA_HIP(hipMemsetAsync(tile + nt, 0, 4, q));
            SA_TRY(rv_exclusive_sum_u32(ws, tile, tile, nt + 1));
            u32 mbig = 0;
            SA_TRY(rv_read_back(ws, &mbig, tile + nt, 4));
            if (mbig > 0) {
                text_big = text_round;
                SA_TRY(need_isa());
                u32 *Pb = bPb.as<u32>(), *Qb = bQb.as<u32>();
                hipLaunchKernelGGL(k_flag_emit, dim3((unsigned)nt), dim3(TB), 0, q, (const uint8_t *)bigflag, m, (const u32 *)tile, (const u32 *)P, (const sav_t *)S,
                                   (const u32 *)G, n, h, (const u32 *)ISA, Pb, Sfree, Qb, kA);
                SA_HIP(hipGetLastError());
                if (!list_in_todo) SA_TRY(leave_fused(Pb, (int64_t)mbig));
                sav_t *sb0 = Sfree, *sb1 = reinterpret_cast<sav_t *>(bseed.p);
                int f1 = 0, f2 = 0;
                SA_TRY(rv_radix_sort_pairs<sav_t>(ws, kA, sb0, kB, sb1, mbig, 0, lowbits, &f1));
                u64 *k_in = f1 ? kB : kA, *k_out = f1 ? kA : kB;
                sav_t *s_in = f1 ? sb1 : sb0, *s_out = f1 ? sb0 : sb1;
                SA_TRY(rv_radix_sort_pairs<sav_t>(ws, k_in, s_in, k_out, s_out, mbig, 32, 32 + highbits, &f2));
                const u64 *kS = f2 ? k_out : k_in;
                const sav_t *sS = f2 ? s_out : s_in;
                s.radix_passes += rv_radix_passes(ws, lowbits) + rv_radix_passes(ws, highbits); s.sorted_elems += mbig;
                hipLaunchKernelGGL(k_big_writeback, dim3((unsigned)ceil_div(mbig, TB)), dim3(TB), 0, q, kS, (const u32 *)Pb, (const u32 *)Qb, sS, (int64_t)mbig, S, head, SA);
                SA_HIP(hipGetLastError());
            }
        }
        int64_t m2 = 0;
        SA_TRY(count_unsorted(head, m, &m2));
        if (far_round) s.far_pairs = (m - m2) / 2;
        if (m2 == 0) break;
        if (!can_far && !can_list) fused = false;
        hipLaunchKernelGGL(k_seed, dim3(mb), dim3(TB), 0, q, (const uint8_t *)head, (const u32 *)P, m, seed);
        SA_HIP(hipGetLastError());
        SA_TRY(rv_inclusive_max_u32(ws, seed, grp, m));
        if (isa_built) {
            hipLaunchKernelGGL(k_round_isa, dim3(mb), dim3(TB), 0, q, (const sav_t *)S, (const u32 *)grp, m, ISA, (const u32 *)G);
            SA_HIP(hipGetLastError());
        }
        if (!Pn) {
            SA_TRY(bP1.reserve((size_t)std::max<int64_t>(m_list0, 1) * 4)); SA_TRY(bG1.reserve((size_t)std::max<int64_t>(m_list0, 1) * 4));
            Pn = bP1.as<u32>(); Gn = bG1.as<u32>();
        }
        const bool want_cls = (text_round && text_big && !ws.opt.no_slow_class && n > 2 * TEXT_LIM) || cls != nullptr;
        if (want_cls) {
            SA_TRY(bcls0.reserve((size_t)m2 + 64)); SA_TRY(bcls1.reserve((size_t)m2 + 64));
            cls_next = (cls == bcls0.as<uint8_t>()) ? bcls1.as<uint8_t>() : bcls0.as<uint8_t>();
            SA_TRY(emit_unsorted(head, m, P, S, grp, Pn, Sfree, Gn, text_round ? (const uint8_t *)bigflag : (const uint8_t *)cls, cls_next, text_round ? 1 : 0));
            cls = cls_next;
        } else
        SA_TRY(emit_unsorted(head, m, P, S, grp, Pn, Sfree, Gn));
        { u32 *t = P; P = Pn; Pn = t; t = G; G = Gn; Gn = t; }
        { sav_t *t = S; S = Sfree; Sfree = t; }
        m = m2;
        if (text_round && !text_big && !ws.opt.no_text_jump && h < TEXT_LIM && n > 2 * TEXT_LIM) h = TEXT_LIM;
        else if (!far_round) h *= 2;
    }
    if (fused && partial) {
        DBuf &bov = ws.sa[29];
        SA_TRY(bov.reserve(64));
        SA_HIP(hipMemsetAsync(bov.p, 0, 4, q));
        hipLaunchKernelGGL(k_lcp_list, dim3((unsigned)ceil_div(ntodo * 64, TB)), dim3(TB), 0, q, T, n, (const sa_t *)SA, (const u32 *)btodo.as<u32>(), ntodo, LCP, BWT, side_sep,
                           d_maxlcp, bov.as<u32>());
        SA_HIP(hipGetLastError());
        u32 ov = 0;
        SA_TRY(rv_read_back(ws, &ov, bov.p, 4));
        if (ov) fused = false;
        s.lcp_list = ntodo;
    }
#undef SA_TRY
#undef SA_HIP
    freeall();
    if (st) *st = s;
    if (fused_done) *fused_done = fused;
    return 0;
}
```

reveal_amd/csrc/rv_prims.hip:

```cpp
#include "rv_common.h"
#include <string.h>

namespace {

constexpr int SCAN_THREADS = 256;
constexpr int SCAN_ITEMS   = 8;
constexpr int SCAN_TILE    = SCAN_THREADS * SCAN_ITEMS;

template <class T> struct OpSum {
    __device__ static T id() { return (T)0; }
    __device__ static T f(T a, T b) { return a + b; }
};
template <class T> struct OpMax {
    __device__ static T id() { return (T)0; }
    __device__ static T f(T a, T b) { return a > b ? a : b; }
};

template <class T> __device__ inline T shfl_up_t(T v, int d) { return __shfl_up(v, d, 64); }
template <> __device__ inline u64 shfl_up_t<u64>(u64 v, int d) {
    u32 lo = __shfl_up((u32)v, d, 64), hi = __shfl_up((u32)(v >> 32), d, 64);
    return ((u64)hi << 32) | lo;
}

template <class T, class Op>
__device__ inline T block_exclusive(T x, T *lds , T *total) {
    const int lane = threadIdx.x & 63, w = threadIdx.x >> 6;
    T inc = x;
#pragma unroll
    for (int d = 1; d < 64; d <<= 1) {
        T t = shfl_up_t<T>(inc, d);
        if (lane >= d) inc = Op::f(t, inc);
    }
    T exc = shfl_up_t<T>(inc, 1);
    if (lane == 0) exc = Op::id();
    if (lane == 63) lds[w] = inc;
    __syncthreads();
    T base = Op::id(), tot = Op::id();
#pragma unroll
    for (int k = 0; k < SCAN_THREADS / 64; k++) {
        T v = lds[k];
        if (k < w) base = Op::f(base, v);
        tot = Op::f(tot, v);
    }
    __syncthreads();
    *total = tot;
    return Op::f(base, exc);
}

template <class T, class Op>
__global__ __launch_bounds__(SCAN_THREADS) void k_tile_reduce(const T *__restrict__ in, T *__restrict__ totals, int64_t n) {
    __shared__ T lds[4];
    const int64_t base = (int64_t)blockIdx.x * SCAN_TILE + (int64_t)threadIdx.x * SCAN_ITEMS;
    T acc = Op::id();
    if (base + SCAN_ITEMS <= n) {
        T v[SCAN_ITEMS];
        __builtin_memcpy(v, in + base, sizeof v);
#pragma unroll
        for (int i = 0; i < SCAN_ITEMS; i++) acc = Op::f(acc, v[i]);
    } else {
#pragma unroll
        for (int i = 0; i < SCAN_ITEMS; i++)
            if (base + i < n) acc = Op::f(acc, in[base + i]);
    }
    T tot;
    (void)block_exclusive<T, Op>(acc, lds, &tot);
    if (threadIdx.x == 0) totals[blockIdx.x] = tot;
}

template <class T, class Op, bool INCL>
__global__ __launch_bounds__(SCAN_THREADS) void k_tile_scan(const T *in, T *out, const T *__restrict__ tile_prefix, int64_t n) {
    __shared__ T lds[4];
    const int64_t base = (int64_t)blockIdx.x * SCAN_TILE + (int64_t)threadIdx.x * SCAN_ITEMS;
    T v[SCAN_ITEMS];
    const bool whole = base + SCAN_ITEMS <= n;
    if (whole) __builtin_memcpy(v, in + base, sizeof v);
    else {
#pragma unroll
        for (int i = 0; i < SCAN_ITEMS; i++) v[i] = (base + i < n) ? in[base + i] : Op::id();
    }
    T acc = Op::id();
#pragma unroll
    for (int i = 0; i < SCAN_ITEMS; i++) acc = Op::f(acc, v[i]);
    T tot;
    T pre = block_exclusive<T, Op>(acc, lds, &tot);
    if (tile_prefix) pre = Op::f(tile_prefix[blockIdx.x], pre);
    if (whole) {
        T o[SCAN_ITEMS];
#pragma unroll
        for (int i = 0; i < SCAN_ITEMS; i++) { const T nx = Op::f(pre, v[i]); o[i] = INCL ? nx : pre; pre = nx; }
        __builtin_memcpy(out + base, o, sizeof o);
        return;
    }
#pragma unroll
    for (int i = 0; i < SCAN_ITEMS; i++) {
        T nx = Op::f(pre, v[i]);
        if (base + i < n) out[base + i] = INCL ? nx : pre;
        pre = nx;
    }
}

template <class T, class Op, bool INCL>
int scan_rec(Workspace &ws, const T *in, T *out, int64_t n, int level) {
    if (n <= 0) return 0;
    const int64_t nt = ceil_div(n, SCAN_TILE);
    if (nt == 1) {
        hipLaunchKernelGGL((k_tile_scan<T, Op, INCL>), dim3(1), dim3(SCAN_THREADS), 0, ws.stream, in, out, (const T *)nullptr, n);
        RV_LAUNCH_CHECK();
        return 0;
    }
    if (level >= 4) { rv_set_error("scan: too many levels"); return -1; }
    RV_TRY(ws.scan_tmp[level].reserve((size_t)nt * sizeof(T)));
    T *tot = ws.scan_tmp[level].as<T>();
    hipLaunchKernelGGL((k_tile_reduce<T, Op>), dim3((unsigned)nt), dim3(SCAN_THREADS), 0, ws.stream, in, tot, n);
    RV_LAUNCH_CHECK();
    RV_TRY((scan_rec<T, Op, false>(ws, tot, tot, nt, level + 1)));
    hipLaunchKernelGGL((k_tile_scan<T, Op, INCL>), dim3((unsigned)nt), dim3(SCAN_THREADS), 0, ws.stream, in, out, (const T *)tot, n);
    RV_LAUNCH_CHECK();
    return 0;
}

}

int rv_exclusive_sum_u32(Workspace &ws, const u32 *in, u32 *out, int64_t n) { return scan_rec<u32, OpSum<u32>, false>(ws, in, out, n, 0); }
int rv_exclusive_sum_u64(Workspace &ws, const u64 *in, u64 *out, int64_t n) { return scan_rec<u64, OpSum<u64>, false>(ws, in, out, n, 0); }
int rv_inclusive_max_u32(Workspace &ws, const u32 *in, u32 *out, int64_t n) { return scan_rec<u32, OpMax<u32>, true>(ws, in, out, n, 0); }
int rv_inclusive_max_u64(Workspace &ws, const u64 *in, u64 *out, int64_t n) { return scan_rec<u64, OpMax<u64>, true>(ws, in, out, n, 0); }

namespace {

#ifndef RV_RS_THREADS
#define RV_RS_THREADS 256
#endif
constexpr int RS_THREADS = RV_RS_THREADS;
#ifndef RV_RS_ITEMS
#define RV_RS_ITEMS 16
#endif
constexpr int RS_ITEMS   = RV_RS_ITEMS;
constexpr int RS_TILE    = RS_THREADS * RS_ITEMS;
constexpr int RS_WAVES   = RS_THREADS / 64;

constexpr unsigned RS_XCDS = 8;
template <bool XCD> __device__ inline u32 rs_tile_of(u32 nb) {
    if (!XCD) return blockIdx.x;
    const u32 chunk = (nb + RS_XCDS - 1) / RS_XCDS;
    return (blockIdx.x % RS_XCDS) * chunk + blockIdx.x / RS_XCDS;
}

template <int BITS, bool XCD>
__global__ __launch_bounds__(RS_THREADS) void k_rs_hist(const u64 *__restrict__ keys, int64_t n, int shift, u32 dmask, u32 *__restrict__ blockhist, u32 nblocks) {
    constexpr int NB = 1 << BITS;
    __shared__ u32 h[NB];
    const u32 tile = rs_tile_of<XCD>(nblocks);
    if (tile >= nblocks) return;
    for (int k = threadIdx.x; k < NB; k += RS_THREADS) h[k] = 0;
    __syncthreads();
    const int64_t base = (int64_t)tile * RS_TILE;
    u64 key[RS_ITEMS];
#pragma unroll
    for (int r = 0; r < RS_ITEMS; r++) {
        const int64_t i = base + (int64_t)r * RS_THREADS + threadIdx.x;
        key[r] = i < n ? keys[i] : 0ull;
    }
#pragma unroll
    for (int r = 0; r < RS_ITEMS; r++) {
        const int64_t i = base + (int64_t)r * RS_THREADS + threadIdx.x;
        if (i < n) atomicAdd(&h[(u32)(key[r] >> shift) & dmask], 1u);
    }
    __syncthreads();
    for (int k = threadIdx.x; k < NB; k += RS_THREADS) blockhist[(size_t)k * nblocks + tile] = h[k];
}

template <bool XCD>
__global__ __launch_bounds__(RS_THREADS) void k_rs_hist_bytes(const uint8_t *__restrict__ digits, int64_t n, u32 *__restrict__ blockhist, u32 nblocks) {
    static_assert(RS_ITEMS == 16, "sixteen digit bytes per thread");
    __shared__ u32 h[256];
    const u32 tile = rs_tile_of<XCD>(nblocks);
    if (tile >= nblocks) return;
    h[threadIdx.x] = 0;
    __syncthreads();
    const int64_t i0 = (int64_t)tile * RS_TILE + (int64_t)threadIdx.x * 16;
    if (i0 + 16 <= n) {
        const uint4 v = *reinterpret_cast<const uint4 *>(digits + i0);
        const u32 w[4] = {v.x, v.y, v.z, v.w};
#pragma unroll
        for (int k = 0; k < 4; k++)
#pragma unroll
            for (int b = 0; b < 4; b++) atomicAdd(&h[(w[k] >> (8 * b)) & 255u], 1u);
    } else {
        for (int64_t i = i0; i < n && i < i0 + 16; i++) atomicAdd(&h[digits[i]], 1u);
    }
    __syncthreads();
    blockhist[(size_t)threadIdx.x * nblocks + tile] = h[threadIdx.x];
}

template <class V, int BITS, bool XCD, class CNT>
__global__ __launch_bounds__(RS_THREADS) void k_rs_scatter(const u64 *__restrict__ kin, const V *__restrict__ vin,
                                                            u64 *__restrict__ kout, V *__restrict__ vout, int64_t n, int shift, u32 dmask,
                                                            const u32 *__restrict__ blockoff, u32 nblocks, uint8_t *__restrict__ dnext, int nshift, u32 nmask) {
    constexpr int NB = 1 << BITS;
    constexpr int BPT = NB / RS_THREADS;
    static_assert(NB % RS_THREADS == 0 && RS_TILE < 65536, "bins per thread, 16-bit counters");
    __shared__ CNT cnt[RS_WAVES][NB];
    __shared__ u32 gbase[NB];
    __shared__ CNT dstart[NB];
    __shared__ u32 wtot[RS_WAVES];
    __shared__ u64 skey[RS_TILE];
    __shared__ V sval[RS_TILE];
    const u32 tile = rs_tile_of<XCD>(nblocks);
    if (tile >= nblocks) return;
    const int lane = threadIdx.x & 63, w = threadIdx.x >> 6;
    for (int k = threadIdx.x; k < RS_WAVES * NB; k += RS_THREADS) (&cnt[0][0])[k] = 0;
    for (int k = threadIdx.x; k < NB; k += RS_THREADS) gbase[k] = blockoff[(size_t)k * nblocks + tile];
    __syncthreads();

    const int64_t wbase = (int64_t)tile * RS_TILE + (int64_t)w * (64 * RS_ITEMS);
    u64 key[RS_ITEMS];
    V val[RS_ITEMS];
    u32 rnk[RS_ITEMS];
    const u64 lt = (lane == 0) ? 0ull : (~0ull >> (64 - lane));
#pragma unroll
    for (int r = 0; r < RS_ITEMS; r++) {
        const int64_t i = wbase + (int64_t)r * 64 + lane;
        key[r] = i < n ? kin[i] : ~0ull;
    }
#pragma unroll
    for (int r = 0; r < RS_ITEMS; r++) {
        const int64_t i = wbase + (int64_t)r * 64 + lane;
        val[r] = i < n ? vin[i] : V(0);
    }
#pragma unroll
    for (int r = 0; r < RS_ITEMS; r++) {
        const int64_t i = wbase + (int64_t)r * 64 + lane;
        const bool valid = i < n;
        const u32 d = (u32)(key[r] >> shift) & dmask;
        u64 peers = __ballot(valid);
#pragma unroll
        for (int b = 0; b < BITS; b++) {
            const bool bit = (d >> b) & 1u;
            const u64 bal = __ballot(bit);
            peers &= bit ? bal : ~bal;
        }
        const u32 below = (u32)__popcll(peers & lt);
        const u32 old = cnt[w][d];
        __builtin_amdgcn_wave_barrier();
        if (valid && below == 0) cnt[w][d] = (CNT)(old + (u32)__popcll(peers));
        __builtin_amdgcn_wave_barrier();
        rnk[r] = old + below;
    }
    __syncthreads();
    u32 tot[BPT], mytot = 0;
#pragma unroll
    for (int b = 0; b < BPT; b++) {
        const int d = threadIdx.x * BPT + b;
        u32 run = 0;
#pragma unroll
        for (int k = 0; k < RS_WAVES; k++) { const u32 c = cnt[k][d]; cnt[k][d] = (CNT)run; run += c; }
        tot[b] = run; mytot += run;
    }
    {
        u32 inc = mytot;
#pragma unroll
        for (int dd = 1; dd < 64; dd <<= 1) { const u32 t = __shfl_up(inc, dd, 64); if (lane >= dd) inc += t; }
        if (lane == 63) wtot[w] = inc;
        __syncthreads();
        u32 before = inc - mytot;
#pragma unroll
        for (int k = 0; k < RS_WAVES; k++) if (k < w) before += wtot[k];
#pragma unroll
        for (int b = 0; b < BPT; b++) { dstart[threadIdx.x * BPT + b] = (CNT)before; before += tot[b]; }
    }
    __syncthreads();
#pragma unroll
    for (int r = 0; r < RS_ITEMS; r++) {
        const int64_t i = wbase + (int64_t)r * 64 + lane;
        if (i < n) {
            const u32 d = (u32)(key[r] >> shift) & dmask;
            const u32 li = (u32)dstart[d] + (u32)cnt[w][d] + rnk[r];
            skey[li] = key[r];
            sval[li] = val[r];
        }
    }
    __syncthreads();
    const int64_t tbase = (int64_t)tile * RS_TILE;
    const u32 nvalid = (u32)((n - tbase) < (int64_t)RS_TILE ? (n - tbase) : (int64_t)RS_TILE);
    for (u32 li = threadIdx.x; li < nvalid; li += RS_THREADS) {
        const u64 k = skey[li];
        const u32 d = (u32)(k >> shift) & dmask;
        const size_t dst = (size_t)gbase[d] + (li - (u32)dstart[d]);
        kout[dst] = k;
        vout[dst] = sval[li];
        if (dnext) dnext[dst] = (uint8_t)((u32)(k >> nshift) & nmask);
    }
}

template <class V, int BITS, bool XCD, class CNT>
static void rs_scatter_launch(hipStream_t q, u32 nb, const u64 *ki, const V *vi, u64 *ko, V *vo, int64_t n, int shift, u32 dmask, const u32 *bh,
                              uint8_t *dnext, int nshift, u32 nmask) {
    const u32 grid = XCD ? RS_XCDS * ((nb + RS_XCDS - 1) / RS_XCDS) : nb;
    hipLaunchKernelGGL((k_rs_scatter<V, BITS, XCD, CNT>), dim3(grid), dim3(RS_THREADS), 0, q, ki, vi, ko, vo, n, shift, dmask, bh, nb, dnext, nshift, nmask);
}

}

int rv_radix_passes(const Workspace &ws, int nbits) {
    const int w = ws.opt.rs_bits == 10 ? 10 : 8;
    return nbits <= 0 ? 0 : (nbits + w - 1) / w;
}

template <class V>
int rv_radix_sort_pairs(Workspace &ws, u64 *k0, V *v0, u64 *k1, V *v1, int64_t n, int bit_lo, int bit_hi, int *result_in_1) {
    *result_in_1 = 0;
    if (n <= 1 || bit_hi <= bit_lo) return 0;
    if (n >= ((int64_t)1 << 32)) { rv_set_error("radix sort: n >= 2^32 not supported"); return -1; }
    const int width = ws.opt.rs_bits == 10 ? 10 : 8;
    const bool xcd = ws.opt.rs_xcd != 0, c16 = ws.opt.rs_cnt16 != 0;
    const u32 nb = (u32)ceil_div(n, RS_TILE);
    RV_TRY(ws.rs_hist.reserve(((size_t)1 << width) * nb * sizeof(u32)));
    u32 *bh = ws.rs_hist.as<u32>();
    const bool bytes = width == 8 && !ws.opt.rs_no_digit_bytes && n >= ((int64_t)1 << 20) && bit_hi - bit_lo > width;
    if (bytes) RV_TRY(ws.rs_digits.reserve((size_t)n + 64));
    uint8_t *dig = bytes ? ws.rs_digits.as<uint8_t>() : nullptr;
    bool have_digits = false;
    u64 *ki = k0, *ko = k1;
    V *vi = v0, *vo = v1;
    int flip = 0;
    for (int shift = bit_lo; shift < bit_hi; shift += width) {
        const int wbits = bit_hi - shift < width ? bit_hi - shift : width;
        const u32 dmask = (1u << wbits) - 1u;
        int pid = ws.prof_begin(8 , (have_digits ? 1.0 : 8.0) * (double)n);
        const u32 hgrid = xcd ? RS_XCDS * ((nb + RS_XCDS - 1) / RS_XCDS) : nb;
        if (have_digits) {
            if (xcd) hipLaunchKernelGGL((k_rs_hist_bytes<true>), dim3(hgrid), dim3(RS_THREADS), 0, ws.stream, (const uint8_t *)dig, n, bh, nb);
            else hipLaunchKernelGGL((k_rs_hist_bytes<false>), dim3(hgrid), dim3(RS_THREADS), 0, ws.stream, (const uint8_t *)dig, n, bh, nb);
        } else if (width == 10) { if (xcd) hipLaunchKernelGGL((k_rs_hist<10, true>), dim3(hgrid), dim3(RS_THREADS), 0, ws.stream, (const u64 *)ki, n, shift, dmask, bh, nb);
                           else hipLaunchKernelGGL((k_rs_hist<10, false>), dim3(hgrid), dim3(RS_THREADS), 0, ws.stream, (const u64 *)ki, n, shift, dmask, bh, nb); }
        else             { if (xcd) hipLaunchKernelGGL((k_rs_hist<8, true>), dim3(hgrid), dim3(RS_THREADS), 0, ws.stream, (const u64 *)ki, n, shift, dmask, bh, nb);
                           else hipLaunchKernelGGL((k_rs_hist<8, false>), dim3(hgrid), dim3(RS_THREADS), 0, ws.stream, (const u64 *)ki, n, shift, dmask, bh, nb); }
        RV_LAUNCH_CHECK();
        ws.prof_end(pid);
        RV_TRY(rv_exclusive_sum_u32(ws, bh, bh, ((int64_t)1 << width) * nb));
        const int nshift = shift + width;
        const bool more = nshift < bit_hi;
        const u32 nmask = more ? ((1u << (bit_hi - nshift < width ? bit_hi - nshift : width)) - 1u) : 0u;
        uint8_t *dn = (bytes && more) ? dig : nullptr;
        pid = ws.prof_begin(7 , (2.0 * (8.0 + sizeof(V)) + (dn ? 1.0 : 0.0)) * (double)n);
#define RS_GO(B_, X_, C_) rs_scatter_launch<V, B_, X_, C_>(ws.stream, nb, (const u64 *)ki, (const V *)vi, ko, vo, n, shift, dmask, (const u32 *)bh, dn, nshift, nmask)
        if (width == 10) { if (xcd) { if (c16) RS_GO(10, true, uint16_t); else RS_GO(10, true, u32); } else { if (c16) RS_GO(10, false, uint16_t); else RS_GO(10, false, u32); } }
        else             { if (xcd) { if (c16) RS_GO(8, true, uint16_t); else RS_GO(8, true, u32); } else { if (c16) RS_GO(8, false, uint16_t); else RS_GO(8, false, u32); } }
#undef RS_GO
        RV_LAUNCH_CHECK();
        ws.prof_end(pid);
        have_digits = dn != nullptr;
        u64 *tk = ki; ki = ko; ko = tk;
        V *tv = vi; vi = vo; vo = tv;
        flip ^= 1;
    }
    *result_in_1 = flip;
    return 0;
}

__global__ __launch_bounds__(256) void k_h2d_copy(const uint4 *__restrict__ src, uint4 *__restrict__ dst, size_t n16) {
    for (size_t i = (size_t)blockIdx.x * 256 + threadIdx.x; i < n16; i += (size_t)gridDim.x * 256) dst[i] = src[i];
}
int rv_read_back(Workspace &ws, void *dst, const void *dsrc, size_t bytes) {
    RV_TRY(ws.hpin.reserve(bytes < 4096 ? 4096 : bytes));
    if (!ws.ev_rb) RV_HIP(hipEventCreateWithFlags(&ws.ev_rb, hipEventDisableTiming));
    RV_HIP(hipMemcpyAsync(ws.hpin.p, dsrc, bytes, hipMemcpyDeviceToHost, ws.stream));
    RV_HIP(hipEventRecord(ws.ev_rb, ws.stream));
    const hipError_t e = rv_event_wait(ws.ev_rb);
    if (e != hipSuccess) { rv_set_error("rv_read_back: %s", hipGetErrorString(e)); return -1; }
    memcpy(dst, ws.hpin.p, bytes);
    return 0;
}

int rv_h2d_copy(Workspace &ws, const void *pinned_src, void *dst, size_t bytes) {
    const size_t n16 = (bytes + 15) / 16;
    if (n16 == 0) return 0;
    size_t blocks = (n16 + 255) / 256;
    if (blocks > 512) blocks = 512;
    hipLaunchKernelGGL(k_h2d_copy, dim3((unsigned)blocks), dim3(256), 0, ws.stream, (const uint4 *)pinned_src, (uint4 *)dst, n16);
    RV_LAUNCH_CHECK();
    return 0;
}

template int rv_radix_sort_pairs<u32>(Workspace &, u64 *, u32 *, u64 *, u32 *, int64_t, int, int, int *);
template int rv_radix_sort_pairs<u64>(Workspace &, u64 *, u64 *, u64 *, u64 *, int64_t, int, int, int *);
```

Baseline: 22490.

## Add hybrid radix sort: two dense-bucket passes plus in-block finish sort

Adds a hybrid radix sort for suffix-array keys. It maps the leading packed symbol fields through a lookup table to a dense 16-bit bucket code, runs two 8-bit scatter passes on that code, then sorts each bucket in a single block with a local rank-and-place kernel. If any bucket exceeds the block capacity, it falls back to the full LSD radix sort. A host-side cost model built from symbol histograms decides whether the hybrid pays off. This aims to replace the many radix passes over wide keys with about three passes, at the cost of extra kernels, a device readback, and a possible fallback that repeats the work.

```diff
diff --git a/include/reveal_amd.h b/include/reveal_amd.h
--- a/include/reveal_amd.h
+++ b/include/reveal_amd.h
@@ -218,6 +218,8 @@
 int rv_test_inclusive_max_u32(const uint32_t *in, uint32_t *out, int64_t n);
 int rv_test_radix_sort(uint64_t *keys, uint32_t *vals, int64_t n, int bit_lo, int bit_hi);
 int rv_test_radix_time(int64_t n, int bits, int dist, int flags, int iters, double *ms, int64_t *bad);
+int rv_test_radix_hybrid(int64_t n, int bits, int dist, int rare_permille, int hybrid, int iters, double *ms, int64_t *bad, int *fell_back,
+                         uint32_t *max_bucket, uint64_t *keys, uint32_t *vals);
 
 #ifdef __cplusplus
 }
diff --git a/reveal_amd/_lib.py b/reveal_amd/_lib.py
--- a/reveal_amd/_lib.py
+++ b/reveal_amd/_lib.py
@@ -165,6 +165,7 @@
     "rv_test_inclusive_max_u32": (_I, [V, V, _L]),
     "rv_test_radix_sort": (_I, [V, V, _L, _I, _I]),
     "rv_test_radix_time": (_I, [_L, _I, _I, _I, _I, ctypes.POINTER(_D), c_i64p]),
+    "rv_test_radix_hybrid": (_I, [_L, _I, _I, _I, _I, _I, ctypes.POINTER(_D), c_i64p, ctypes.POINTER(_I), ctypes.POINTER(ctypes.c_uint32), V, V]),
 }
 
 
diff --git a/reveal_amd/csrc/rv_api.hip b/reveal_amd/csrc/rv_api.hip
--- a/reveal_amd/csrc/rv_api.hip
+++ b/reveal_amd/csrc/rv_api.hip
@@ -1170,3 +1170,88 @@
 }
 
 }
+namespace {
+__global__ __launch_bounds__(256) void k_rt_fill_fields(u64 *keys, u32 *vals, int64_t n, int bits, int dist, u32 rare_permille) {
+    const int64_t i = (int64_t)blockIdx.x * 256 + threadIdx.x;
+    if (i >= n) return;
+    const u64 r = rt_mix((u64)i * 0x9E3779B97F4A7C15ull + 12345);
+    u64 k = 0;
+    if (dist == 2) k = r;
+    else if (dist != 3) {
+        u64 r2 = rt_mix(r), r3 = rt_mix(r2 ^ 0x5bd1e995ull);
+        for (int f = 0; f < 9; f++) {
+            u32 v = 0;
+            for (int e = 0; e < 3; e++) {
+                u32 sym = 1u + (u32)(r2 & 3); r2 >>= 2;
+                if ((u32)(r3 & 1023) * 1000u < rare_permille * 1024u) sym = 0;
+                r3 = (r3 >> 10) | (r3 << 54); if (e == 2) r3 = rt_mix(r3);
+                if (dist == 1 && (i & 1) && f * 3 + e < 9) sym = 2;
+                v = v * 5 + sym;
+            }
+            k = (k << 7) | v;
+        }
+        k >>= (63 - bits);
+    }
+    const u64 mask = bits >= 64 ? ~0ull : (1ull << bits) - 1;
+    keys[i] = (k & mask) | (r & ~mask & 0x00ffffffffffffffull);
+    vals[i] = (u32)i;
+}
+__global__ __launch_bounds__(256) void k_rt_iota(u32 *vals, int64_t n) {
+    const int64_t i = (int64_t)blockIdx.x * 256 + threadIdx.x;
+    if (i < n) vals[i] = (u32)i;
+}
+}
+extern "C" {
+int rv_test_radix_hybrid(int64_t n, int bits, int dist, int rare_permille, int hybrid, int iters, double *ms, int64_t *bad, int *fell_back,
+                         uint32_t *max_bucket, uint64_t *keys, uint32_t *vals) {
+    if (n <= 0 || bits < 35 || bits > 56 || iters < 1) { rv_set_error("rv_test_radix_hybrid: n >= 1, 35 <= bits <= 56, iters >= 1"); return -1; }
+    Workspace ws;
+    RV_TRY(test_ws(ws));
+    RvKeyFields kf; kf.g = 3; kf.fb = 7; kf.nf = bits / 7 + 1; kf.bits = bits; kf.rad = 5;
+    ws.rs_finish_alt = hybrid == 2;
+    u64 cc[5] = {(u64)rare_permille * 4, (u64)(1000 - rare_permille), (u64)(1000 - rare_permille), (u64)(1000 - rare_permille), (u64)(1000 - rare_permille)};
+    const u64 *ccp = dist == 2 ? nullptr : cc;
+    if (keys) {
+        for (int c = 0; c < 5; c++) cc[c] = 0;
+        for (int64_t i = 0; i < n; i++) { const u32 v = (u32)(keys[i] >> (bits - 7)) & 127u; if (v < 125) { cc[v / 25]++; cc[v / 5 % 5]++; cc[v % 5]++; } }
+        ccp = cc;
+    }
+    DBuf k0, k1, v0, v1, db;
+    int r = 0, in1 = 0, fb = 0;
+    u32 mb = 0;
+    hipEvent_t e0 = nullptr, e1 = nullptr;
+    if (k0.reserve((size_t)n * 8 + 64) || k1.reserve((size_t)n * 8 + 64) || v0.reserve((size_t)n * 4 + 64) || v1.reserve((size_t)n * 4 + 64) || db.reserve(64)) r = -1;
+    if (!r && (hipEventCreate(&e0) != hipSuccess || hipEventCreate(&e1) != hipSuccess)) r = -1;
+    for (int it = 0; !r && it < iters; it++) {
+        if (keys) {
+            if (hipMemcpyAsync(k0.p, keys, (size_t)n * 8, hipMemcpyHostToDevice, ws.stream) != hipSuccess) { r = -1; break; }
+            hipLaunchKernelGGL(k_rt_iota, dim3((unsigned)ceil_div(n, 256)), dim3(256), 0, ws.stream, v0.as<u32>(), n);
+        } else hipLaunchKernelGGL(k_rt_fill_fields, dim3((unsigned)ceil_div(n, 256)), dim3(256), 0, ws.stream, k0.as<u64>(), v0.as<u32>(), n, bits, dist, (u32)rare_permille);
+        (void)hipEventRecord(e0, ws.stream);
+        if (hybrid) r = rv_radix_sort_hybrid<u32>(ws, k0.as<u64>(), v0.as<u32>(), k1.as<u64>(), v1.as<u32>(), n, kf, ccp, &in1, &fb, &mb);
+        else r = rv_radix_sort_pairs<u32>(ws, k0.as<u64>(), v0.as<u32>(), k1.as<u64>(), v1.as<u32>(), n, 0, bits, &in1);
+        (void)hipEventRecord(e1, ws.stream);
+        if (!r && hipEventSynchronize(e1) != hipSuccess) { rv_set_error("sync failed: %s", hipGetErrorString(hipGetLastError())); r = -1; }
+        float t = 0;
+        if (!r && ms) { (void)hipEventElapsedTime(&t, e0, e1); ms[it] = t; }
+    }
+    if (!r) {
+        (void)hipMemsetAsync(db.p, 0, 8, ws.stream);
+        hipLaunchKernelGGL(k_rt_check, dim3((unsigned)ceil_div(n, 256)), dim3(256), 0, ws.stream, (const u64 *)(in1 ? k1.p : k0.p), (const u32 *)(in1 ? v1.p : v0.p), n, bits,
+                           db.as<unsigned long long>());
+        unsigned long long b = 0;
+        if (hipMemcpyAsync(&b, db.p, 8, hipMemcpyDeviceToHost, ws.stream) != hipSuccess || hipStreamSynchronize(ws.stream) != hipSuccess) r = -1;
+        if (bad) *bad = (int64_t)b;
+        if (!r && keys && hipMemcpy(keys, in1 ? k1.p : k0.p, (size_t)n * 8, hipMemcpyDeviceToHost) != hipSuccess) r = -1;
+        if (!r && vals && hipMemcpy(vals, in1 ? v1.p : v0.p, (size_t)n * 4, hipMemcpyDeviceToHost) != hipSuccess) r = -1;
+    }
+    if (fell_back) *fell_back = fb;
+    if (max_bucket) *max_bucket = mb;
+    if (e0) (void)hipEventDestroy(e0);
+    if (e1) (void)hipEventDestroy(e1);
+    k0.release(); k1.release(); v0.release(); v1.release(); db.release();
+    test_ws_done(ws);
+    return r;
+}
+
+}
diff --git a/reveal_amd/csrc/rv_common.h b/reveal_amd/csrc/rv_common.h
--- a/reveal_amd/csrc/rv_common.h
+++ b/reveal_amd/csrc/rv_common.h
@@ -86,6 +86,7 @@
     X(rs_xcd, "RV_RS_XCD", 1) \
     X(rs_cnt16, "RV_RS_CNT16", 1) \
     X(rs_no_digit_bytes, "RV_RS_NO_DIGIT_BYTES", 0) \
+    X(rs_hybrid, "RV_RS_HYBRID", -1) \
     X(diag_table, "RV_DIAG_TABLE", -1) \
     X(no_cascade_chain, "RV_NO_CASCADE_CHAIN", 0) \
     X(casm_rank_count, "RV_CASM_RANK_COUNT", 0) \
@@ -291,6 +292,8 @@
     DBuf scan_tmp[4];
     DBuf rs_hist;
     DBuf rs_digits;
+    DBuf rs_aux;
+    int rs_finish_alt = 0;
     DBuf misc[20];
     DBuf sa[32];
     HBuf hpin;
@@ -310,7 +313,7 @@
         hpin.release();
         if (ev_rb) { (void)hipEventDestroy(ev_rb); ev_rb = nullptr; }
         for (auto &b : scan_tmp) b.release();
-        rs_hist.release(); rs_digits.release();
+        rs_hist.release(); rs_digits.release(); rs_aux.release();
         for (auto &b : misc) b.release();
         for (auto &b : sa) b.release();
     }
@@ -332,6 +335,14 @@
 template <class V>
 int rv_radix_sort_pairs(Workspace &ws, u64 *k0, V *v0, u64 *k1, V *v1, int64_t n,
                         int bit_lo, int bit_hi, int *result_in_1);
+
+struct RvKeyFields { int g, fb, nf, bits; u32 rad; };
+constexpr int RV_RSH_CAP = 6144;
+bool rv_rs_hybrid_possible(const Workspace &ws, const RvKeyFields &kf, int64_t n);
+bool rv_rs_hybrid_pays(const RvKeyFields &kf, const u64 *code_count, int64_t n);
+template <class V>
+int rv_radix_sort_hybrid(Workspace &ws, u64 *k0, V *v0, u64 *k1, V *v1, int64_t n, const RvKeyFields &kf, const u64 *code_count,
+                         int *result_in_1, int *fell_back, u32 *max_bucket);
 
 int rv_read_back(Workspace &ws, void *dst, const void *dsrc, size_t bytes);
 
diff --git a/reveal_amd/csrc/rv_construct.hip b/reveal_amd/csrc/rv_construct.hip
--- a/reveal_amd/csrc/rv_construct.hip
+++ b/reveal_amd/csrc/rv_construct.hip
@@ -2339,8 +2339,23 @@
     }
     SA_HIP(hipGetLastError());
     int in1 = 0;
-    SA_TRY(rv_radix_sort_pairs<sav_t>(ws, bk0.as<u64>(), bv0.as<sav_t>(), bk1.as<u64>(), bv1.as<sav_t>(), nsort, 0, bits, &in1));
-    s.radix_passes += rv_radix_passes(ws, bits); s.sorted_elems += nsort;
+    bool hybrid = false;
+    RvKeyFields kf; kf.g = kp.g; kf.fb = kp.fb; kf.nf = kp.nf; kf.bits = bits; kf.rad = radix;
+    u64 code_count[256];
+    if (ws.opt.rs_hybrid != 0 && rv_rs_hybrid_possible(ws, kf, nsort)) {
+        for (u32 c = 0; c < 256; c++) code_count[c] = 0;
+        for (int c = 0; c < 256; c++) if (hist[c] && lut[c] < radix) code_count[lut[c]] += hist[c];
+        hybrid = ws.opt.rs_hybrid == 1 || rv_rs_hybrid_pays(kf, code_count, nsort);
+    }
+    if (hybrid) {
+        int fell_back = 0;
+        SA_TRY(rv_radix_sort_hybrid<sav_t>(ws, bk0.as<u64>(), bv0.as<sav_t>(), bk1.as<u64>(), bv1.as<sav_t>(), nsort, kf, code_count, &in1, &fell_back, nullptr));
+        s.radix_passes += fell_back ? rv_radix_passes(ws, bits) : 3;
+    } else {
+        SA_TRY(rv_radix_sort_pairs<sav_t>(ws, bk0.as<u64>(), bv0.as<sav_t>(), bk1.as<u64>(), bv1.as<sav_t>(), nsort, 0, bits, &in1));
+        s.radix_passes += rv_radix_passes(ws, bits);
+    }
+    s.sorted_elems += nsort;
     u64 *ks = in1 ? bk1.as<u64>() : bk0.as<u64>();
     sav_t *vs = in1 ? bv1.as<sav_t>() : bv0.as<sav_t>();
     u64 *kt = in1 ? bk0.as<u64>() : bk1.as<u64>();
diff --git a/reveal_amd/csrc/rv_prims.hip b/reveal_amd/csrc/rv_prims.hip
--- a/reveal_amd/csrc/rv_prims.hip
+++ b/reveal_amd/csrc/rv_prims.hip
@@ -1,5 +1,7 @@
 #include "rv_common.h"
 #include <string.h>
+#include <vector>
+#include <algorithm>
 
 namespace {
 
@@ -146,13 +148,44 @@
     return (blockIdx.x % RS_XCDS) * chunk + blockIdx.x / RS_XCDS;
 }
 
-template <int BITS, bool XCD>
-__global__ __launch_bounds__(RS_THREADS) void k_rs_hist(const u64 *__restrict__ keys, int64_t n, int shift, u32 dmask, u32 *__restrict__ blockhist, u32 nblocks) {
+struct RsPlain {
+    static constexpr bool dense = false;
+    int shift; u32 dmask; int nshift; u32 nmask;
+    __device__ u32 cur(u64 k, const uint8_t *) const { return (u32)(k >> shift) & dmask; }
+    __device__ void both(u64 k, const uint8_t *, u32 *d, u32 *dn) const { *d = (u32)(k >> shift) & dmask; *dn = (u32)(k >> nshift) & nmask; }
+    __device__ void stage(uint8_t *) const {}
+};
+constexpr int RSD_TAB = 512;
+struct RsDense {
+    static constexpr bool dense = true;
+    const uint8_t *tab; int top, fb, g2, nfd, drop, hi; u32 fmask;
+    __device__ void stage(uint8_t *stab) const { for (int k = threadIdx.x; k < RSD_TAB; k += blockDim.x) stab[k] = tab[k]; }
+    __device__ u32 bucket(u64 k, const uint8_t *stab) const {
+        const u32 cm = (1u << g2) - 1u;
+        u32 acc = 0, st = 0;
+        int sh = top;
+        for (int f = 0; f < nfd; f++) {
+            sh -= fb;
+            const u32 t = stab[(u32)(k >> sh) & fmask];
+            const u32 c = st == 0 ? (t & cm) : (st == 1 ? 0u : cm);
+            st = st ? st : (t >> 6);
+            acc = (acc << g2) | c;
+        }
+        return (acc >> drop) & 0xffffu;
+    }
+    __device__ u32 cur(u64 k, const uint8_t *stab) const { const u32 b = bucket(k, stab); return hi ? b >> 8 : b & 255u; }
+    __device__ void both(u64 k, const uint8_t *stab, u32 *d, u32 *dn) const { const u32 b = bucket(k, stab); *d = hi ? b >> 8 : b & 255u; *dn = hi ? b & 255u : b >> 8; }
+};
+
+template <int BITS, bool XCD, class DG>
+__global__ __launch_bounds__(RS_THREADS) void k_rs_hist(const u64 *__restrict__ keys, int64_t n, DG dg, u32 *__restrict__ blockhist, u32 nblocks) {
     constexpr int NB = 1 << BITS;
     __shared__ u32 h[NB];
+    __shared__ uint8_t stab[DG::dense ? RSD_TAB : 1];
     const u32 tile = rs_tile_of<XCD>(nblocks);
     if (tile >= nblocks) return;
     for (int k = threadIdx.x; k < NB; k += RS_THREADS) h[k] = 0;
+    dg.stage(stab);
     __syncthreads();
     const int64_t base = (int64_t)tile * RS_TILE;
     u64 key[RS_ITEMS];
@@ -164,7 +197,7 @@
 #pragma unroll
     for (int r = 0; r < RS_ITEMS; r++) {
         const int64_t i = base + (int64_t)r * RS_THREADS + threadIdx.x;
-        if (i < n) atomicAdd(&h[(u32)(key[r] >> shift) & dmask], 1u);
+        if (i < n) atomicAdd(&h[dg.cur(key[r], stab)], 1u);
     }
     __syncthreads();
     for (int k = threadIdx.x; k < NB; k += RS_THREADS) blockhist[(size_t)k * nblocks + tile] = h[k];
@@ -193,10 +226,10 @@
     blockhist[(size_t)threadIdx.x * nblocks + tile] = h[threadIdx.x];
 }
 
-template <class V, int BITS, bool XCD, class CNT>
+template <class V, int BITS, bool XCD, class CNT, class DG>
 __global__ __launch_bounds__(RS_THREADS) void k_rs_scatter(const u64 *__restrict__ kin, const V *__restrict__ vin,
-                                                            u64 *__restrict__ kout, V *__restrict__ vout, int64_t n, int shift, u32 dmask,
-                                                            const u32 *__restrict__ blockoff, u32 nblocks, uint8_t *__restrict__ dnext, int nshift, u32 nmask) {
+                                                            u64 *__restrict__ kout, V *__restrict__ vout, int64_t n, DG dg,
+                                                            const u32 *__restrict__ blockoff, u32 nblocks, uint8_t *__restrict__ dnext) {
     constexpr int NB = 1 << BITS;
     constexpr int BPT = NB / RS_THREADS;
     static_assert(NB % RS_THREADS == 0 && RS_TILE < 65536, "bins per thread, 16-bit counters");
@@ -206,9 +239,11 @@
     __shared__ u32 wtot[RS_WAVES];
     __shared__ u64 skey[RS_TILE];
     __shared__ V sval[RS_TILE];
+    __shared__ uint8_t stab[DG::dense ? RSD_TAB : 1];
     const u32 tile = rs_tile_of<XCD>(nblocks);
     if (tile >= nblocks) return;
     const int lane = threadIdx.x & 63, w = threadIdx.x >> 6;
+    dg.stage(stab);
     for (int k = threadIdx.x; k < RS_WAVES * NB; k += RS_THREADS) (&cnt[0][0])[k] = 0;
     for (int k = threadIdx.x; k < NB; k += RS_THREADS) gbase[k] = blockoff[(size_t)k * nblocks + tile];
     __syncthreads();
@@ -217,6 +252,7 @@
     u64 key[RS_ITEMS];
     V val[RS_ITEMS];
     u32 rnk[RS_ITEMS];
+    u32 dig[DG::dense ? RS_ITEMS : 1];
     const u64 lt = (lane == 0) ? 0ull : (~0ull >> (64 - lane));
 #pragma unroll
     for (int r = 0; r < RS_ITEMS; r++) {
@@ -232,7 +268,8 @@
     for (int r = 0; r < RS_ITEMS; r++) {
         const int64_t i = wbase + (int64_t)r * 64 + lane;
         const bool valid = i < n;
-        const u32 d = (u32)(key[r] >> shift) & dmask;
+        const u32 d = dg.cur(key[r], stab);
+        if (DG::dense) dig[r] = d;
         u64 peers = __ballot(valid);
 #pragma unroll
         for (int b = 0; b < BITS; b++) {
@@ -274,7 +311,7 @@
     for (int r = 0; r < RS_ITEMS; r++) {
         const int64_t i = wbase + (int64_t)r * 64 + lane;
         if (i < n) {
-            const u32 d = (u32)(key[r] >> shift) & dmask;
+            const u32 d = DG::dense ? dig[DG::dense ? r : 0] : dg.cur(key[r], stab);
             const u32 li = (u32)dstart[d] + (u32)cnt[w][d] + rnk[r];
             skey[li] = key[r];
             sval[li] = val[r];
@@ -285,19 +322,19 @@
     const u32 nvalid = (u32)((n - tbase) < (int64_t)RS_TILE ? (n - tbase) : (int64_t)RS_TILE);
     for (u32 li = threadIdx.x; li < nvalid; li += RS_THREADS) {
         const u64 k = skey[li];
-        const u32 d = (u32)(k >> shift) & dmask;
+        u32 d, dn;
+        dg.both(k, stab, &d, &dn);
         const size_t dst = (size_t)gbase[d] + (li - (u32)dstart[d]);
         kout[dst] = k;
         vout[dst] = sval[li];
-        if (dnext) dnext[dst] = (uint8_t)((u32)(k >> nshift) & nmask);
-    }
-}
-
-template <class V, int BITS, bool XCD, class CNT>
-static void rs_scatter_launch(hipStream_t q, u32 nb, const u64 *ki, const V *vi, u64 *ko, V *vo, int64_t n, int shift, u32 dmask, const u32 *bh,
-                              uint8_t *dnext, int nshift, u32 nmask) {
+        if (dnext) dnext[dst] = (uint8_t)dn;
+    }
+}
+
+template <class V, int BITS, bool XCD, class CNT, class DG>
+static void rs_scatter_launch(hipStream_t q, u32 nb, const u64 *ki, const V *vi, u64 *ko, V *vo, int64_t n, DG dg, const u32 *bh, uint8_t *dnext) {
     const u32 grid = XCD ? RS_XCDS * ((nb + RS_XCDS - 1) / RS_XCDS) : nb;
-    hipLaunchKernelGGL((k_rs_scatter<V, BITS, XCD, CNT>), dim3(grid), dim3(RS_THREADS), 0, q, ki, vi, ko, vo, n, shift, dmask, bh, nb, dnext, nshift, nmask);
+    hipLaunchKernelGGL((k_rs_scatter<V, BITS, XCD, CNT, DG>), dim3(grid), dim3(RS_THREADS), 0, q, ki, vi, ko, vo, n, dg, bh, nb, dnext);
 }
 
 }
@@ -327,24 +364,25 @@
     for (int shift = bit_lo; shift < bit_hi; shift += width) {
         const int wbits = bit_hi - shift < width ? bit_hi - shift : width;
         const u32 dmask = (1u << wbits) - 1u;
+        const int nshift = shift + width;
+        const bool more = nshift < bit_hi;
+        const u32 nmask = more ? ((1u << (bit_hi - nshift < width ? bit_hi - nshift : width)) - 1u) : 0u;
+        const RsPlain pdg{shift, dmask, nshift, nmask};
         int pid = ws.prof_begin(8 , (have_digits ? 1.0 : 8.0) * (double)n);
         const u32 hgrid = xcd ? RS_XCDS * ((nb + RS_XCDS - 1) / RS_XCDS) : nb;
         if (have_digits) {
             if (xcd) hipLaunchKernelGGL((k_rs_hist_bytes<true>), dim3(hgrid), dim3(RS_THREADS), 0, ws.stream, (const uint8_t *)dig, n, bh, nb);
             else hipLaunchKernelGGL((k_rs_hist_bytes<false>), dim3(hgrid), dim3(RS_THREADS), 0, ws.stream, (const uint8_t *)dig, n, bh, nb);
-        } else if (width == 10) { if (xcd) hipLaunchKernelGGL((k_rs_hist<10, true>), dim3(hgrid), dim3(RS_THREADS), 0, ws.stream, (const u64 *)ki, n, shift, dmask, bh, nb);
-                           else hipLaunchKernelGGL((k_rs_hist<10, false>), dim3(hgrid), dim3(RS_THREADS), 0, ws.stream, (const u64 *)ki, n, shift, dmask, bh, nb); }
-        else             { if (xcd) hipLaunchKernelGGL((k_rs_hist<8, true>), dim3(hgrid), dim3(RS_THREADS), 0, ws.stream, (const u64 *)ki, n, shift, dmask, bh, nb);
-                           else hipLaunchKernelGGL((k_rs_hist<8, false>), dim3(hgrid), dim3(RS_THREADS), 0, ws.stream, (const u64 *)ki, n, shift, dmask, bh, nb); }
+        } else if (width == 10) { if (xcd) hipLaunchKernelGGL((k_rs_hist<10, true, RsPlain>), dim3(hgrid), dim3(RS_THREADS), 0, ws.stream, (const u64 *)ki, n, pdg, bh, nb);
+                           else hipLaunchKernelGGL((k_rs_hist<10, false, RsPlain>), dim3(hgrid), dim3(RS_THREADS), 0, ws.stream, (const u64 *)ki, n, pdg, bh, nb); }
+        else             { if (xcd) hipLaunchKernelGGL((k_rs_hist<8, true, RsPlain>), dim3(hgrid), dim3(RS_THREADS), 0, ws.stream, (const u64 *)ki, n, pdg, bh, nb);
+                           else hipLaunchKernelGGL((k_rs_hist<8, false, RsPlain>), dim3(hgrid), dim3(RS_THREADS), 0, ws.stream, (const u64 *)ki, n, pdg, bh, nb); }
         RV_LAUNCH_CHECK();
         ws.prof_end(pid);
         RV_TRY(rv_exclusive_sum_u32(ws, bh, bh, ((int64_t)1 << width) * nb));
-        const int nshift = shift + width;
-        const bool more = nshift < bit_hi;
-        const u32 nmask = more ? ((1u << (bit_hi - nshift < width ? bit_hi - nshift : width)) - 1u) : 0u;
         uint8_t *dn = (bytes && more) ? dig : nullptr;
         pid = ws.prof_begin(7 , (2.0 * (8.0 + sizeof(V)) + (dn ? 1.0 : 0.0)) * (double)n);
-#define RS_GO(B_, X_, C_) rs_scatter_launch<V, B_, X_, C_>(ws.stream, nb, (const u64 *)ki, (const V *)vi, ko, vo, n, shift, dmask, (const u32 *)bh, dn, nshift, nmask)
+#define RS_GO(B_, X_, C_) rs_scatter_launch<V, B_, X_, C_, RsPlain>(ws.stream, nb, (const u64 *)ki, (const V *)vi, ko, vo, n, pdg, (const u32 *)bh, dn)
         if (width == 10) { if (xcd) { if (c16) RS_GO(10, true, uint16_t); else RS_GO(10, true, u32); } else { if (c16) RS_GO(10, false, uint16_t); else RS_GO(10, false, u32); } }
         else             { if (xcd) { if (c16) RS_GO(8, true, uint16_t); else RS_GO(8, true, u32); } else { if (c16) RS_GO(8, false, uint16_t); else RS_GO(8, false, u32); } }
 #undef RS_GO
@@ -359,6 +397,327 @@
     return 0;
 }
 
+namespace {
+constexpr int RSF_CAP = RV_RSH_CAP;
+constexpr u32 RSF_MAXBIN = 1024;
+constexpr u32 RSB_NONE = 0xffffffffu;
+constexpr int64_t RSH_MIN_N = (int64_t)1 << 27;
+static_assert(RSF_CAP < 65536, "16-bit places");
+enum { RSI_FAIL = 0, RSI_MAXB = 1, RSI_SPANS = 2, RSI_WORDS = 16 };
+
+__global__ __launch_bounds__(256) void k_rs_bucket_starts(const uint8_t *__restrict__ dig, int64_t n, const u32 *__restrict__ bh, u32 nb, u32 *__restrict__ starts) {
+    __shared__ u32 s_d1[256];
+    s_d1[threadIdx.x] = bh[(size_t)threadIdx.x * nb];
+    __syncthreads();
+    const int64_t i0 = ((int64_t)blockIdx.x * 256 + threadIdx.x) * 16;
+    if (i0 >= n) return;
+    u32 w[4] = {0, 0, 0, 0};
+    if (i0 + 16 <= n) { const uint4 v = *reinterpret_cast<const uint4 *>(dig + i0); w[0] = v.x; w[1] = v.y; w[2] = v.z; w[3] = v.w; }
+    else for (int64_t i = i0; i < n; i++) w[(i - i0) >> 2] |= (u32)dig[i] << (8 * ((i - i0) & 3));
+    u32 prev = i0 > 0 ? (u32)dig[i0 - 1] : 0x100u;
+#pragma unroll
+    for (int j = 0; j < 16; j++) {
+        const u32 c = (w[j >> 2] >> (8 * (j & 3))) & 255u;
+        const int64_t i = i0 + j;
+        if (i < n && c != prev) {
+            int lo = 0, hi = 255;
+            while (lo < hi) { const int mid = (lo + hi + 1) >> 1; if ((int64_t)s_d1[mid] <= i) lo = mid; else hi = mid - 1; }
+            starts[lo * 256 + (int)c] = (u32)i;
+        }
+        prev = c;
+    }
+}
+
+__global__ __launch_bounds__(256) void k_rs_spans(const uint8_t *__restrict__ dig, int64_t n, const u32 *__restrict__ bh, u32 nb, const u32 *__restrict__ starts,
+                                                  uint2 *__restrict__ spans, u32 *__restrict__ info, u32 cap) {
+    __shared__ u32 s_st[257], s_sz[256], s_max, s_bad, s_ns;
+    __shared__ uint2 s_sp[256];
+    const u32 d = blockIdx.x, e = threadIdx.x;
+    const u32 lo = bh[(size_t)d * nb], hi = d < 255 ? bh[(size_t)(d + 1) * nb] : (u32)n;
+    if (lo >= hi) { spans[d * 256 + e] = make_uint2(0, 0); return; }
+    const u32 e0 = dig[lo];
+    const u32 s = e == e0 ? lo : starts[d * 256 + e];
+    s_st[e] = s;
+    if (e == 0) { s_st[256] = hi; s_max = 0; s_bad = 0; s_ns = 0; }
+    __syncthreads();
+    u32 z = 0;
+    if (s != RSB_NONE) {
+        u32 j = e + 1;
+        while (s_st[j] == RSB_NONE) j++;
+        const u32 nx = s_st[j];
+        if (nx < s || s < lo || nx > hi) s_bad = 1; else z = nx - s;
+        atomicMax(&s_max, z);
+    }
+    s_sz[e] = z;
+    __syncthreads();
+    if (e == 0) {
+        u32 ns = 0, cs = 0, cz = 0;
+        for (int k = 0; k < 256; k++) {
+            const u32 zk = s_sz[k];
+            if (!zk) continue;
+            if (cz && cz + zk > cap) { s_sp[ns++] = make_uint2(cs, cz); cz = 0; }
+            if (!cz) cs = s_st[k];
+            cz += zk;
+        }
+        if (cz) s_sp[ns++] = make_uint2(cs, cz);
+        s_ns = ns;
+        atomicMax(info + RSI_MAXB, s_max);
+        atomicAdd(info + RSI_SPANS, ns);
+        if (s_max > cap || s_bad) atomicOr(info + RSI_FAIL, 1u);
+    }
+    __syncthreads();
+    spans[d * 256 + e] = e < s_ns ? s_sp[e] : make_uint2(0, 0);
+}
+
+__device__ inline u64 rsf_shfl_xor(u64 v, int m) {
+    const u32 lo = __shfl_xor((u32)v, m, 64), hi = __shfl_xor((u32)(v >> 32), m, 64);
+    return ((u64)hi << 32) | lo;
+}
+
+template <class V, int RSF_THREADS>
+__global__ __launch_bounds__(RSF_THREADS, (sizeof(V) == 4 || RSF_THREADS == 1024) ? 4 : 2) void k_rs_finish(const u64 *__restrict__ kin, const V *__restrict__ vin, u64 *__restrict__ kout, V *__restrict__ vout,
+                                                            const uint2 *__restrict__ spans, u64 mask, u32 *__restrict__ info) {
+    constexpr int RSF_IPT = RSF_CAP / RSF_THREADS, RSF_BINS = 8 * RSF_THREADS, RSF_BPT = 8;
+    static_assert(RSF_CAP % RSF_THREADS == 0, "items per thread");
+    constexpr int RAW = (RSF_CAP * 2 + RSF_BINS * 4) > RSF_CAP * (int)sizeof(V) ? (RSF_CAP * 2 + RSF_BINS * 4) : RSF_CAP * (int)sizeof(V);
+    __shared__ u64 skey[RSF_CAP];
+    __shared__ __align__(16) unsigned char sraw[RAW];
+    __shared__ u64 s_min[RSF_THREADS / 64], s_max[RSF_THREADS / 64], s_mul, s_lo;
+    __shared__ u32 s_wsum[RSF_THREADS / 64], s_bad;
+    __shared__ int s_sh;
+    const uint2 sp = spans[blockIdx.x];
+    const u32 m = sp.y;
+    if (m == 0) return;
+    if (__builtin_nontemporal_load(info + RSI_FAIL)) return;
+    if (m > (u32)RSF_CAP) { if (threadIdx.x == 0) atomicOr(info + RSI_FAIL, 1u); return; }
+    const size_t base = sp.x;
+    uint16_t *perm = reinterpret_cast<uint16_t *>(sraw);
+    u32 *bins = reinterpret_cast<u32 *>(sraw + RSF_CAP * 2);
+    V *sval = reinterpret_cast<V *>(sraw);
+    const int t = threadIdx.x, lane = t & 63, w = t >> 6;
+
+    u64 key[RSF_IPT];
+    V val[RSF_IPT];
+    u64 kmin = ~0ull, kmax = 0ull;
+#pragma unroll
+    for (int i = 0; i < RSF_IPT; i++) { const u32 r = t + i * RSF_THREADS; key[i] = r < m ? kin[base + r] : 0ull; }
+#pragma unroll
+    for (int i = 0; i < RSF_IPT; i++) { const u32 r = t + i * RSF_THREADS; val[i] = r < m ? vin[base + r] : V(0); }
+#pragma unroll
+    for (int k = 0; k < RSF_BPT; k++) bins[t + k * RSF_THREADS] = 0;
+#pragma unroll
+    for (int i = 0; i < RSF_IPT; i++) {
+        const u32 r = t + i * RSF_THREADS;
+        if (r < m) { const u64 mk = key[i] & mask; kmin = mk < kmin ? mk : kmin; kmax = mk > kmax ? mk : kmax; skey[r] = key[i]; }
+    }
+#pragma unroll
+    for (int d = 1; d < 64; d <<= 1) {
+        const u64 a = rsf_shfl_xor(kmin, d), b = rsf_shfl_xor(kmax, d);
+        kmin = a < kmin ? a : kmin; kmax = b > kmax ? b : kmax;
+    }
+    if (lane == 0) { s_min[w] = kmin; s_max[w] = kmax; }
+    __syncthreads();
+    if (t == 0) {
+        u64 lo = ~0ull, hi = 0ull;
+        for (int k = 0; k < RSF_THREADS / 64; k++) { lo = s_min[k] < lo ? s_min[k] : lo; hi = s_max[k] > hi ? s_max[k] : hi; }
+        const u64 range = hi - lo;
+        const int bl = range ? 64 - __builtin_clzll(range) : 0;
+        const int sh = bl > 24 ? bl - 24 : 0;
+        s_lo = lo; s_sh = sh; s_bad = 0;
+        s_mul = ((u64)RSF_BINS << 32) / ((range >> sh) + 1ull);
+    }
+    __syncthreads();
+    const u64 klo = s_lo, mul = s_mul;
+    const int sh = s_sh;
+    u32 bin[RSF_IPT], rnk[RSF_IPT];
+#pragma unroll
+    for (int i = 0; i < RSF_IPT; i++) {
+        const u32 r = t + i * RSF_THREADS;
+        bin[i] = 0; rnk[i] = 0;
+        if (r < m) {
+            bin[i] = (u32)(((((key[i] & mask) - klo) >> sh) * mul) >> 32);
+            rnk[i] = atomicAdd(&bins[bin[i]], 1u);
+        }
+    }
+    __syncthreads();
+    {
+        uint4 a = reinterpret_cast<uint4 *>(bins)[2 * t], b = reinterpret_cast<uint4 *>(bins)[2 * t + 1];
+        u32 c[8] = {a.x, a.y, a.z, a.w, b.x, b.y, b.z, b.w};
+        u32 sum = 0, big = 0;
+#pragma unroll
+        for (int k = 0; k < 8; k++) { sum += c[k]; big = c[k] > big ? c[k] : big; }
+        if (big > RSF_MAXBIN) s_bad = 1;
+        u32 inc = sum;
+#pragma unroll
+        for (int d = 1; d < 64; d <<= 1) { const u32 x = __shfl_up(inc, d, 64); if (lane >= d) inc += x; }
+        if (lane == 63) s_wsum[w] = inc;
+        __syncthreads();
+        u32 run = inc - sum;
+        for (int k = 0; k < w; k++) run += s_wsum[k];
+#pragma unroll
+        for (int k = 0; k < 8; k++) { const u32 x = c[k]; c[k] = run; run += x; }
+        reinterpret_cast<uint4 *>(bins)[2 * t] = make_uint4(c[0], c[1], c[2], c[3]);
+        reinterpret_cast<uint4 *>(bins)[2 * t + 1] = make_uint4(c[4], c[5], c[6], c[7]);
+    }
+    __syncthreads();
+    if (s_bad) { if (t == 0) atomicOr(info + RSI_FAIL, 1u); return; }
+#pragma unroll
+    for (int i = 0; i < RSF_IPT; i++) {
+        const u32 r = t + i * RSF_THREADS;
+        if (r < m) perm[bins[bin[i]] + rnk[i]] = (uint16_t)r;
+    }
+    __syncthreads();
+#pragma unroll
+    for (int i = 0; i < RSF_IPT; i++) {
+        const u32 r = t + i * RSF_THREADS;
+        if (r < m) {
+            const u32 s = bins[bin[i]], e = bin[i] + 1 < (u32)RSF_BINS ? bins[bin[i] + 1] : m;
+            const u64 mk = key[i] & mask;
+            u32 cnt = 0;
+            for (u32 j = s; j < e; j++) {
+                const u32 r2 = perm[j];
+                const u64 k2 = skey[r2] & mask;
+                cnt += (k2 < mk || (k2 == mk && r2 < r)) ? 1u : 0u;
+            }
+            rnk[i] = s + cnt;
+        }
+    }
+    __syncthreads();
+#pragma unroll
+    for (int i = 0; i < RSF_IPT; i++) {
+        const u32 r = t + i * RSF_THREADS;
+        if (r < m) { skey[rnk[i]] = key[i]; sval[rnk[i]] = val[i]; }
+    }
+    __syncthreads();
+    for (u32 j = t; j < m; j += RSF_THREADS) { kout[base + j] = skey[j]; vout[base + j] = sval[j]; }
+}
+
+struct RsParts { int ngroups; std::vector<int> grp; int mainm[4]; double pmax, rare; };
+static RsParts rs_partition(const RvKeyFields &kf, const u64 *code_count) {
+    const int R = (int)kf.rad;
+    std::vector<double> c(R, 1.0), pre(R + 1, 0.0);
+    if (code_count) { double tot = 0; for (int k = 0; k < R; k++) tot += (double)code_count[k]; if (tot > 0) for (int k = 0; k < R; k++) c[k] = (double)code_count[k]; }
+    for (int k = 0; k < R; k++) pre[k + 1] = pre[k] + c[k];
+    RsParts P;
+    P.ngroups = R < 4 ? R : 4;
+    const int G = P.ngroups;
+    std::vector<std::vector<double>> best(G + 1, std::vector<double>(R + 1, 1e300));
+    std::vector<std::vector<int>> cut(G + 1, std::vector<int>(R + 1, 0));
+    best[0][0] = 0;
+    for (int k = 1; k <= G; k++)
+        for (int i = k; i <= R; i++)
+            for (int j = k - 1; j < i; j++) {
+                const double v = std::max(best[k - 1][j], pre[i] - pre[j]);
+                if (v < best[k][i]) { best[k][i] = v; cut[k][i] = j; }
+            }
+    P.grp.assign(R, 0);
+    int end = R;
+    for (int k = G; k >= 1; k--) { const int j = cut[k][end]; for (int x = j; x < end; x++) P.grp[x] = k - 1; end = j; }
+    for (int k = 0; k < 4; k++) P.mainm[k] = -1;
+    for (int x = 0; x < R; x++) { const int k = P.grp[x]; if (P.mainm[k] < 0 || c[x] > c[P.mainm[k]]) P.mainm[k] = x; }
+    const double tot = pre[R] > 0 ? pre[R] : 1.0;
+    P.pmax = best[G][R] / tot; P.rare = 0;
+    for (int x = 0; x < R; x++) if (x != P.mainm[P.grp[x]]) P.rare = std::max(P.rare, c[x] / tot);
+    return P;
+}
+}
+
+bool rv_rs_hybrid_possible(const Workspace &ws, const RvKeyFields &kf, int64_t n) {
+    return ws.opt.rs_bits != 10 && ws.opt.rs_xcd != 0 && ws.opt.rs_cnt16 != 0 && kf.g >= 1 && kf.g <= 3 && kf.fb >= 1 && (1 << kf.fb) <= RSD_TAB &&
+           (kf.nf - 1) * kf.g >= 8 && kf.bits <= 63 && kf.bits >= (kf.nf - 1) * kf.fb && kf.rad >= 2 && n >= 2 && n < ((int64_t)1 << 32);
+}
+bool rv_rs_hybrid_pays(const RvKeyFields &kf, const u64 *code_count, int64_t n) {
+    if (n < RSH_MIN_N) return false;
+    const RsParts P = rs_partition(kf, code_count);
+    double p8 = 1; for (int k = 0; k < 8; k++) p8 *= P.pmax;
+    return (double)n * std::max(p8, P.rare) * 1.1 <= (double)RSF_CAP;
+}
+
+template <class V>
+int rv_radix_sort_hybrid(Workspace &ws, u64 *k0, V *v0, u64 *k1, V *v1, int64_t n, const RvKeyFields &kf, const u64 *code_count,
+                         int *result_in_1, int *fell_back, u32 *max_bucket) {
+    *result_in_1 = 0;
+    if (fell_back) *fell_back = 0;
+    if (max_bucket) *max_bucket = 0;
+    if (n <= 1) return 0;
+    if (!rv_rs_hybrid_possible(ws, kf, n)) { rv_set_error("hybrid radix sort: key layout or switches not supported"); return -1; }
+    const RsParts P = rs_partition(kf, code_count);
+    uint8_t tab[RSD_TAB];
+    u32 rg = 1; for (int e = 0; e < kf.g; e++) rg *= kf.rad;
+    for (u32 v = 0; v < (u32)RSD_TAB; v++) {
+        u32 code = 0, st = 0;
+        if (v >= rg) { code = (1u << (2 * kf.g)) - 1u; st = 2; }
+        else {
+            u32 div = rg;
+            for (int e = 0; e < kf.g; e++) {
+                div /= kf.rad;
+                const int sym = (int)((v / div) % kf.rad);
+                u32 c;
+                if (st == 0) { c = (u32)P.grp[sym]; if (sym != P.mainm[P.grp[sym]]) st = sym < P.mainm[P.grp[sym]] ? 1 : 2; }
+                else c = st == 1 ? 0u : 3u;
+                code = (code << 2) | c;
+            }
+        }
+        tab[v] = (uint8_t)(code | (st << 6));
+    }
+    const size_t off_info = RSD_TAB, off_starts = 1024, off_spans = off_starts + 65536 * 4;
+    RV_TRY(ws.rs_aux.reserve(off_spans + 65536 * 8));
+    uint8_t *aux = ws.rs_aux.as<uint8_t>();
+    u32 *info = reinterpret_cast<u32 *>(aux + off_info), *starts = reinterpret_cast<u32 *>(aux + off_starts);
+    uint2 *spans = reinterpret_cast<uint2 *>(aux + off_spans);
+    RV_HIP(hipMemcpyAsync(aux, tab, RSD_TAB, hipMemcpyHostToDevice, ws.stream));
+    RV_HIP(hipMemsetAsync(info, 0, RSI_WORDS * 4, ws.stream));
+    RV_HIP(hipMemsetAsync(starts, 0xff, 65536 * 4, ws.stream));
+    const u32 nb = (u32)ceil_div(n, RS_TILE);
+    RV_TRY(ws.rs_hist.reserve((size_t)256 * nb * sizeof(u32)));
+    RV_TRY(ws.rs_digits.reserve((size_t)n + 64));
+    u32 *bh = ws.rs_hist.as<u32>();
+    uint8_t *dig = ws.rs_digits.as<uint8_t>();
+    const u32 grid = RS_XCDS * ((nb + RS_XCDS - 1) / RS_XCDS);
+    RsDense dg;
+    dg.tab = aux; dg.top = kf.bits; dg.fb = kf.fb; dg.g2 = 2 * kf.g; dg.nfd = (8 + kf.g - 1) / kf.g; dg.drop = dg.g2 * dg.nfd - 16; dg.hi = 0; dg.fmask = (1u << kf.fb) - 1u;
+    u64 *ki = k0, *ko = k1;
+    V *vi = v0, *vo = v1;
+    for (int pass = 0; pass < 2; pass++) {
+        dg.hi = pass;
+        int pid = ws.prof_begin(8 , (pass ? 1.0 : 8.0) * (double)n);
+        if (pass) hipLaunchKernelGGL((k_rs_hist_bytes<true>), dim3(grid), dim3(RS_THREADS), 0, ws.stream, (const uint8_t *)dig, n, bh, nb);
+        else hipLaunchKernelGGL((k_rs_hist<8, true, RsDense>), dim3(grid), dim3(RS_THREADS), 0, ws.stream, (const u64 *)ki, n, dg, bh, nb);
+        RV_LAUNCH_CHECK();
+        ws.prof_end(pid);
+        RV_TRY(rv_exclusive_sum_u32(ws, bh, bh, (int64_t)256 * nb));
+        pid = ws.prof_begin(7 , (2.0 * (8.0 + sizeof(V)) + 1.0) * (double)n);
+        rs_scatter_launch<V, 8, true, uint16_t, RsDense>(ws.stream, nb, (const u64 *)ki, (const V *)vi, ko, vo, n, dg, (const u32 *)bh, dig);
+        RV_LAUNCH_CHECK();
+        ws.prof_end(pid);
+        u64 *tk = ki; ki = ko; ko = tk;
+        V *tv = vi; vi = vo; vo = tv;
+    }
+    int pid = ws.prof_begin(8 , (double)n);
+    hipLaunchKernelGGL(k_rs_bucket_starts, dim3((unsigned)ceil_div(n, 256 * 16)), dim3(256), 0, ws.stream, (const uint8_t *)dig, n, (const u32 *)bh, nb, starts);
+    RV_LAUNCH_CHECK();
+    hipLaunchKernelGGL(k_rs_spans, dim3(256), dim3(256), 0, ws.stream, (const uint8_t *)dig, n, (const u32 *)bh, nb, (const u32 *)starts, spans, info, (u32)RSF_CAP);
+    RV_LAUNCH_CHECK();
+    ws.prof_end(pid);
+    const u64 mask = kf.bits >= 64 ? ~0ull : (1ull << kf.bits) - 1ull;
+    pid = ws.prof_begin(7 , 2.0 * (8.0 + sizeof(V)) * (double)n);
+    if (ws.rs_finish_alt) hipLaunchKernelGGL((k_rs_finish<V, 512>), dim3(65536), dim3(512), 0, ws.stream, (const u64 *)ki, (const V *)vi, ko, vo, (const uint2 *)spans, mask, info);
+    else hipLaunchKernelGGL((k_rs_finish<V, 1024>), dim3(65536), dim3(1024), 0, ws.stream, (const u64 *)ki, (const V *)vi, ko, vo, (const uint2 *)spans, mask, info);
+    RV_LAUNCH_CHECK();
+    ws.prof_end(pid);
+    u32 res[3] = {0, 0, 0};
+    RV_TRY(rv_read_back(ws, res, info, sizeof res));
+    if (max_bucket) *max_bucket = res[RSI_MAXB];
+    if (res[RSI_FAIL]) {
+        if (fell_back) *fell_back = 1;
+        return rv_radix_sort_pairs<V>(ws, k0, v0, k1, v1, n, 0, kf.bits, result_in_1);
+    }
+    *result_in_1 = 1;
+    return 0;
+}
+template int rv_radix_sort_hybrid<u32>(Workspace &, u64 *, u32 *, u64 *, u32 *, int64_t, const RvKeyFields &, const u64 *, int *, int *, u32 *);
+template int rv_radix_sort_hybrid<u64>(Workspace &, u64 *, u64 *, u64 *, u64 *, int64_t, const RvKeyFields &, const u64 *, int *, int *, u32 *);
+
 __global__ __launch_bounds__(256) void k_h2d_copy(const uint4 *__restrict__ src, uint4 *__restrict__ dst, size_t n16) {
     for (size_t i = (size_t)blockIdx.x * 256 + threadIdx.x; i < n16; i += (size_t)gridDim.x * 256) dst[i] = src[i];
 }
```

After: 16870. 25.0% lower.
